# emilk/field_interpolation

Measured on AMD Instinct MI355X. Metric: solved lattice points/sec (assembly+CG to field within 1e-5 of the CPU reference by the solver's estimate: ended at rel. residual 1.1e-08), higher is better.
Workload: dtype f64

## Files before the change

field_interpolation_amd/_capi.py:

```python
import ctypes as C
import os

HERE = os.path.dirname(os.path.abspath(__file__))
LIB_PATH = os.environ.get("FI_HIP_LIB", os.path.join(HERE, "libfi_hip.so"))

FI_OK = 0
FI_HOST, FI_DEVICE = 0, 1
FI_F32, FI_F64 = 0, 1
ERR_NAMES = {1: "FI_ERR_INVALID", 2: "FI_ERR_HIP", 3: "FI_ERR_STATE", 4: "FI_ERR_COMM",
             5: "FI_ERR_UNSUPPORTED", 6: "FI_ERR_BREAKDOWN", 7: "FI_ERR_TIMEOUT"}

SYMBOLS = [
    "fi_last_error", "fi_device_count", "fi_ctx_create", "fi_ctx_create_slab", "fi_ctx_destroy",
    "fi_slab_range", "fi_slab_point_range", "fi_slab_partition", "fi_halo_width", "fi_comm_unique_id", "fi_comm_init", "fi_comm_init_host", "fi_comm_info", "fi_comm_self_test", "fi_set_model", "fi_add_points", "fi_add_border_prior",
    "fi_add_rows_coo", "fi_assemble", "fi_clear_points", "fi_set_option", "fi_solve_cg", "fi_jacobi", "fi_tile_pass", "fi_error_map",
    "fi_get_solution_f64", "fi_true_residual", "fi_apply_AtA_f64", "fi_get_Atb_f64", "fi_get_diag_f64",
    "fi_get_stats", "fi_memory_pool", "fi_time_apply", "fi_upscale_field",
    "fi_group_create", "fi_group_destroy", "fi_group_size", "fi_group_rank", "fi_group_assemble",
    "fi_group_solve_cg", "fi_group_apply_AtA_f64", "fi_group_true_residual", "fi_group_get_solution_f64", "fi_group_tile_pass", "fi_group_error_map",
    "fi_group_iso_extract", "fi_iso_extract", "fi_iso_extract_field", "fi_mesh_info", "fi_mesh_copy", "fi_mesh_destroy",
    "fi_dual_contour", "fi_dual_contour_field",
    "fi_mesh_create", "fi_mesh_parts", "fi_mesh_measure", "fi_mesh_select", "fi_mesh_simplify",
    "fi_mesh_smooth", "fi_mesh_normals", "fi_mesh_sample", "fi_mesh_deviation", "fi_mesh_register", "fi_points_register",
    "fi_group_sample", "fi_sample", "fi_sample_field",
    "fi_nearest", "fi_distance_field", "fi_points_create", "fi_points_nearest", "fi_points_distance_field", "fi_points_destroy",
    "fi_knn", "fi_points_knn", "fi_estimate_normals", "fi_points_estimate_normals",
    "fi_orient_normals", "fi_points_orient_normals",
    "fi_radius_count", "fi_points_radius_count", "fi_neighbour_distances", "fi_points_neighbour_distances",
    "fi_outliers_statistical", "fi_points_outliers_statistical", "fi_outliers_radius", "fi_points_outliers_radius", "fi_cloud_thin",
    "fi_cluster", "fi_points_cluster", "fi_cluster_measure", "fi_plane_fit", "fi_planes_segment",
    "fi_points_describe", "fi_feature_match", "fi_align_correspondences",
    "fi_surface_create", "fi_surface_from_mesh", "fi_surface_distance", "fi_surface_distance_field", "fi_surface_destroy",
    "fi_surface_raycast", "fi_surface_count_hits", "fi_surface_contains", "fi_surface_signed_distance",
    "fi_surface_signed_distance_field",
    "fi_redistance", "fi_redistance_field",
    "fi_point_count", "fi_point_residuals", "fi_robust_reweight", "fi_reset_point_weights", "fi_solve_robust",
]
FI_LOSS = {"huber": 0, "cauchy": 1, "tukey": 2}
FI_LOSS_NONE = -1
FI_REGISTER = {"plane": 0, "point": 1}
FI_THIN = {"mean": 0, "first": 1}


class FiWeights(C.Structure):
    _fields_ = [("data_pos", C.c_float), ("data_gradient", C.c_float),
                ("model_0", C.c_float), ("model_1", C.c_float), ("model_2", C.c_float),
                ("model_3", C.c_float), ("model_4", C.c_float), ("gradient_smoothness", C.c_float),
                ("value_kernel", C.c_int), ("gradient_kernel", C.c_int)]


class FiSolveOptions(C.Structure):
    _fields_ = [("tile", C.c_int), ("tile_size", C.c_int), ("cg", C.c_int),
                ("max_iterations", C.c_int), ("error_tolerance", C.c_float)]


class FiTriplet(C.Structure):
    _fields_ = [("row", C.c_int), ("col", C.c_int), ("value", C.c_float)]


class FiStats(C.Structure):
    _fields_ = [("num_unknowns", C.c_long), ("num_data_rows", C.c_long), ("num_cells", C.c_long),
                ("num_generic_rows", C.c_long), ("iterations", C.c_int), ("converged", C.c_int),
                ("rel_residual", C.c_double), ("assemble_ms", C.c_double), ("solve_ms", C.c_double),
                ("spmv_ms_avg", C.c_double), ("spmv_samples", C.c_int), ("spmv_bytes", C.c_double),
                ("restarts", C.c_int), ("verified_residual", C.c_double),
                ("num_levels", C.c_int), ("coarse_iterations", C.c_int),
                ("prec_ms_avg", C.c_double), ("prec_samples", C.c_int), ("prec_bytes", C.c_double),
                ("operator_applies", C.c_int), ("halo_exchanges", C.c_int), ("reductions", C.c_int),
                ("coarse_unconverged", C.c_int), ("field_estimate", C.c_double), ("field_per_residual", C.c_double),
                ("stop_residual", C.c_double), ("field_rounds", C.c_int)]


class FiRobustOptions(C.Structure):
    _fields_ = [("loss", C.c_int), ("tuning", C.c_float), ("scale", C.c_float), ("rounds", C.c_int),
                ("weight_tolerance", C.c_float)]


class FiRobustStats(C.Structure):
    _fields_ = [("rounds", C.c_int), ("iterations", C.c_int), ("scale", C.c_float), ("max_weight_change", C.c_float),
                ("points_used", C.c_long), ("points_zeroed", C.c_long), ("reweight_ms", C.c_double)]


class FiMeshPart(C.Structure):
    _fields_ = [("vertices", C.c_longlong), ("primitives", C.c_longlong), ("edges", C.c_longlong),
                ("boundary", C.c_longlong), ("irregular", C.c_longlong), ("size", C.c_double), ("enclosed", C.c_double),
                ("lo", C.c_float * 3), ("hi", C.c_float * 3)]


class FiSmoothOptions(C.Structure):
    _fields_ = [("iterations", C.c_int), ("lam", C.c_float), ("mu", C.c_float), ("boundary", C.c_int),
                ("max_move", C.c_float), ("normals", C.c_int)]


class FiDeviation(C.Structure):
    _fields_ = [("queries", C.c_longlong), ("counted", C.c_longlong), ("beyond", C.c_longlong), ("invalid", C.c_longlong),
                ("at", C.c_longlong), ("max", C.c_double), ("mean", C.c_double), ("rms", C.c_double), ("where", C.c_float * 3)]


class FiRegisterOptions(C.Structure):
    _fields_ = [("mode", C.c_int), ("max_iterations", C.c_int), ("max_distance", C.c_float), ("rotation_tolerance", C.c_double),
# ... 8 lines not shown


class FiOutlierStats(C.Structure):
    _fields_ = [("counted", C.c_long), ("kept", C.c_long), ("mean", C.c_double), ("stddev", C.c_double), ("threshold", C.c_double)]


class FiClusterStats(C.Structure):
    _fields_ = [("clusters", C.c_long), ("core", C.c_long), ("border", C.c_long), ("noise", C.c_long), ("non_finite", C.c_long)]


class FiClusterRow(C.Structure):
    _fields_ = [("count", C.c_long), ("core", C.c_long), ("lo", C.c_float * 3), ("hi", C.c_float * 3), ("centroid", C.c_double * 3)]


class FiPlaneOptions(C.Structure):
    _fields_ = [("threshold", C.c_float), ("max_trials", C.c_long), ("confidence", C.c_double), ("refine", C.c_int),
                ("seed", C.c_ulonglong), ("axis", C.c_float * 3), ("min_cos", C.c_float)]


class FiPlaneModel(C.Structure):
    _fields_ = [("found", C.c_int), ("refits", C.c_int), ("inliers", C.c_long), ("candidates", C.c_long), ("trials", C.c_long),
                ("normal", C.c_double * 3), ("offset", C.c_double), ("rms", C.c_double)]


class FiAlignOptions(C.Structure):
    _fields_ = [("threshold", C.c_float), ("similarity", C.c_float), ("max_trials", C.c_long), ("confidence", C.c_double),
                ("seed", C.c_ulonglong)]


class FiAlignment(C.Structure):
    _fields_ = [("found", C.c_int), ("pairs", C.c_long), ("live", C.c_long), ("trials", C.c_long), ("valid", C.c_long),
                ("inliers", C.c_long), ("transform", C.c_double * 16), ("rms", C.c_double)]


class FiError(RuntimeError):
    def __init__(self, code, msg):
        super().__init__("%s: %s" % (ERR_NAMES.get(code, "error %d" % code), msg))
        self.code = code


_LIB = None


def lib():
    global _LIB
    if _LIB is not None:
        return _LIB
    if not os.path.exists(LIB_PATH):
        raise ImportError("field_interpolation_amd: %s is missing -- run `python -m field_interpolation_amd.build` "
                          "(hipcc, gfx950).  There is no CPU fallback." % LIB_PATH)
    L = C.CDLL(LIB_PATH)
    vp, ip, fp, dp = C.c_void_p, C.POINTER(C.c_int), C.c_void_p, C.POINTER(C.c_double)
    L.fi_last_error.restype = C.c_char_p
    L.fi_device_count.argtypes = [ip]
    L.fi_ctx_create.argtypes = [C.POINTER(vp), C.c_int, ip, C.c_int]
    L.fi_ctx_create_slab.argtypes = [C.POINTER(vp), C.c_int, ip, C.c_int, C.c_int, C.c_int]
    L.fi_ctx_destroy.argtypes = [vp]
    L.fi_slab_range.argtypes = [vp, ip, ip]
    L.fi_slab_point_range.argtypes = [vp, C.POINTER(C.c_float), C.POINTER(C.c_float)]
    L.fi_slab_partition.argtypes = [C.c_int, C.c_int, C.c_int, ip, ip]
    L.fi_halo_width.argtypes = [C.POINTER(FiWeights), ip]
    L.fi_comm_unique_id.argtypes = [vp]
    L.fi_comm_init.argtypes = [vp, vp]
    L.fi_comm_info.argtypes = [vp, C.POINTER(C.c_long)]
    L.fi_comm_init_host.argtypes = [vp, C.c_char_p, C.c_int]
    L.fi_set_model.argtypes = [vp, C.POINTER(FiWeights)]
    L.fi_add_points.argtypes = [vp, C.c_long, fp, fp, fp, fp, C.c_float, C.c_int, C.c_float, C.c_int, C.c_int]
    L.fi_add_border_prior.argtypes = [vp, C.c_float]
    L.fi_add_rows_coo.argtypes = [vp, C.c_long, C.c_long, vp, fp, C.c_int]
    L.fi_assemble.argtypes = [vp]
    L.fi_clear_points.argtypes = [vp]
    L.fi_solve_cg.argtypes = [vp, fp, C.c_int, C.c_float, fp, ip, C.POINTER(C.c_float), C.c_int]
    L.fi_set_option.argtypes = [vp, C.c_int, C.c_double]
    L.fi_jacobi.argtypes = [vp, fp, C.c_int, C.c_float, fp, C.c_int]
    L.fi_tile_pass.argtypes = [vp, fp, C.c_int, fp, C.c_int]
    L.fi_comm_self_test.argtypes = [C.c_int, C.c_long]
    L.fi_error_map.argtypes = [vp, fp, fp, C.c_int]
    L.fi_get_solution_f64.argtypes = [vp, dp]
    L.fi_true_residual.argtypes = [vp, dp]
    L.fi_apply_AtA_f64.argtypes = [vp, dp, dp]
    L.fi_get_Atb_f64.argtypes = [vp, dp]
    L.fi_get_diag_f64.argtypes = [vp, dp]
    L.fi_get_stats.argtypes = [vp, C.POINTER(FiStats)]
    L.fi_time_apply.argtypes = [vp, C.c_int, dp]
    L.fi_memory_pool.argtypes = [C.c_longlong, C.POINTER(C.c_longlong)]
    L.fi_upscale_field.argtypes = [fp, C.c_int, ip, ip, fp, C.c_int]
    L.fi_group_create.argtypes = [C.POINTER(vp), C.c_int, ip, C.c_int, C.c_int]
    L.fi_group_destroy.argtypes = [vp]
    L.fi_group_size.argtypes = [vp]
    L.fi_group_rank.restype = vp
    L.fi_group_rank.argtypes = [vp, C.c_int]
    L.fi_group_assemble.argtypes = [vp]
    L.fi_group_solve_cg.argtypes = [vp, fp, C.c_int, C.c_float, fp, ip, C.POINTER(C.c_float)]
    L.fi_group_apply_AtA_f64.argtypes = [vp, dp, dp]
    L.fi_group_true_residual.argtypes = [vp, dp]
    L.fi_group_get_solution_f64.argtypes = [vp, dp]
    L.fi_group_tile_pass.argtypes = [vp, fp, C.c_int, fp]
    L.fi_group_error_map.argtypes = [vp, fp, fp]
    L.fi_group_iso_extract.argtypes = [vp, fp, C.c_float, C.POINTER(vp)]
    L.fi_iso_extract.argtypes = [vp, fp, C.c_float, C.c_int, C.POINTER(vp)]
    L.fi_iso_extract_field.argtypes = [fp, C.c_int, ip, C.c_float, C.c_int, C.POINTER(vp)]
    L.fi_dual_contour.argtypes = [vp, fp, fp, C.c_float, C.c_int, C.POINTER(vp)]
    L.fi_dual_contour_field.argtypes = [fp, fp, C.c_int, ip, C.c_float, C.c_int, C.POINTER(vp)]
    L.fi_mesh_info.argtypes = [vp, C.POINTER(C.c_long), C.POINTER(C.c_long), ip]
    L.fi_mesh_copy.argtypes = [vp, fp, fp, vp, vp, C.c_int]
    L.fi_mesh_destroy.argtypes = [vp]
    L.fi_mesh_create.argtypes = [C.POINTER(vp), C.c_int, C.c_long, fp, fp, vp, C.c_long, vp, C.c_int]
    L.fi_mesh_parts.argtypes = [vp, C.POINTER(C.c_long), vp, vp, C.c_int]
    L.fi_mesh_measure.argtypes = [vp, C.c_long, vp, C.POINTER(C.c_long)]
    L.fi_mesh_select.argtypes = [vp, C.c_long, vp, C.POINTER(vp)]
    L.fi_mesh_simplify.argtypes = [vp, C.c_float, vp, C.c_int, vp, C.c_int, C.POINTER(vp)]
    L.fi_mesh_smooth.argtypes = [vp, C.POINTER(FiSmoothOptions), C.POINTER(vp)]
    L.fi_mesh_normals.argtypes = [vp, C.POINTER(vp)]
    L.fi_mesh_sample.argtypes = [vp, C.c_long, C.c_ulonglong, C.c_int, fp, fp, vp, C.c_int]
    L.fi_mesh_deviation.argtypes = [vp, vp, C.c_long, C.c_ulonglong, C.c_float, C.POINTER(FiDeviation), C.POINTER(FiDeviation), fp,
                                    C.c_int]
    L.fi_mesh_register.argtypes = [vp, vp, C.c_long, fp, C.POINTER(FiRegisterOptions), dp, C.POINTER(FiRegistration), fp, fp, C.c_int]
    L.fi_points_register.argtypes = [vp, fp, C.c_long, fp, C.POINTER(FiRegisterOptions), dp, C.POINTER(FiRegistration), fp, fp,
                                     C.c_int]
    L.fi_group_sample.argtypes = [vp, fp, C.c_long, fp, C.c_int, C.c_float, fp, fp]
    L.fi_sample.argtypes = [vp, fp, C.c_long, fp, C.c_int, C.c_float, fp, fp, C.c_int]
    L.fi_sample_field.argtypes = [fp, C.c_int, ip, C.c_long, fp, C.c_int, C.c_float, fp, fp, C.c_int]
    L.fi_nearest.argtypes = [vp, C.c_long, fp, C.c_float, fp, vp, C.c_int]
    L.fi_distance_field.argtypes = [vp, C.c_float, fp, vp, C.c_int]
    L.fi_points_create.argtypes = [C.POINTER(vp), C.c_int, C.c_long, fp, C.c_int]
    L.fi_points_nearest.argtypes = [vp, C.c_long, fp, C.c_float, fp, vp, C.c_int]
    L.fi_points_distance_field.argtypes = [vp, ip, C.c_float, fp, vp, C.c_int]
    L.fi_points_destroy.argtypes = [vp]
    L.fi_knn.argtypes = [vp, C.c_long, fp, C.c_int, C.c_float, fp, vp, C.c_int]
    L.fi_points_knn.argtypes = [vp, C.c_long, fp, C.c_int, C.c_float, fp, vp, C.c_int]
    L.fi_estimate_normals.argtypes = [vp, C.c_int, C.c_float, C.c_int, fp, C.c_long, fp, fp, C.c_int]
    L.fi_points_estimate_normals.argtypes = [vp, C.c_int, C.c_float, C.c_int, fp, C.c_long, fp, fp, C.c_int]
    L.fi_orient_normals.argtypes = [vp, C.c_int, C.c_float, C.c_int, fp, C.c_long, fp, vp, C.c_int]
    L.fi_points_orient_normals.argtypes = [vp, C.c_int, C.c_float, C.c_int, fp, C.c_long, fp, vp, C.c_int]
    L.fi_radius_count.argtypes = [vp, C.c_long, fp, C.c_float, C.c_int, vp, C.c_int]
    L.fi_points_radius_count.argtypes = [vp, C.c_long, fp, C.c_float, C.c_int, vp, C.c_int]
    L.fi_neighbour_distances.argtypes = [vp, C.c_int, C.c_float, fp, fp, vp, C.c_int]
    L.fi_points_neighbour_distances.argtypes = [vp, C.c_int, C.c_float, fp, fp, vp, C.c_int]
    L.fi_outliers_statistical.argtypes = [vp, C.c_int, C.c_float, C.c_float, vp, C.POINTER(FiOutlierStats), C.c_int]
    L.fi_points_outliers_statistical.argtypes = [vp, C.c_int, C.c_float, C.c_float, vp, C.POINTER(FiOutlierStats), C.c_int]
    L.fi_outliers_radius.argtypes = [vp, C.c_float, C.c_int, vp, C.POINTER(C.c_long), C.c_int]
    L.fi_points_outliers_radius.argtypes = [vp, C.c_float, C.c_int, vp, C.POINTER(C.c_long), C.c_int]
    L.fi_cloud_thin.argtypes = [C.c_int, C.c_long, fp, fp, fp, C.c_float, C.POINTER(C.c_float), C.c_int, fp, fp, fp, vp, vp, vp,
                                C.POINTER(C.c_long), C.c_int]
    L.fi_cluster.argtypes = [vp, C.c_float, C.c_int, vp, vp, C.POINTER(FiClusterStats), C.c_int]
    L.fi_points_cluster.argtypes = [vp, C.c_float, C.c_int, vp, vp, C.POINTER(FiClusterStats), C.c_int]
    L.fi_cluster_measure.argtypes = [C.c_int, C.c_long, fp, vp, vp, C.c_long, C.POINTER(FiClusterRow), C.c_int]
    L.fi_plane_fit.argtypes = [C.c_int, C.c_long, fp, vp, C.POINTER(FiPlaneOptions), C.POINTER(FiPlaneModel), vp, C.c_int]
    L.fi_planes_segment.argtypes = [C.c_int, C.c_long, fp, vp, C.POINTER(FiPlaneOptions), C.c_int, C.c_long, vp,
                                    C.POINTER(FiPlaneModel), ip, C.c_int]
    L.fi_points_describe.argtypes = [vp, fp, C.c_int, C.c_float, fp, vp, C.c_int]
    L.fi_feature_match.argtypes = [C.c_int, C.c_long, fp, vp, C.c_long, fp, vp, vp, fp, C.c_int]
    L.fi_align_correspondences.argtypes = [C.c_long, fp, C.c_long, fp, C.c_long, vp, vp, C.POINTER(FiAlignOptions),
                                           C.POINTER(FiAlignment), vp, C.c_int]
    L.fi_surface_create.argtypes = [C.POINTER(vp), C.c_int, C.c_long, fp, C.c_long, vp, C.c_int]
    L.fi_surface_from_mesh.argtypes = [C.POINTER(vp), vp]
    L.fi_surface_distance.argtypes = [vp, C.c_long, fp, C.c_float, fp, vp, fp, C.c_int]
    L.fi_surface_distance_field.argtypes = [vp, ip, C.c_float, fp, vp, C.c_int]
    L.fi_surface_destroy.argtypes = [vp]
    L.fi_surface_raycast.argtypes = [vp, C.c_long, fp, fp, C.c_float, C.c_float, fp, vp, fp, C.c_int]
    L.fi_surface_count_hits.argtypes = [vp, C.c_long, fp, fp, C.c_float, C.c_float, C.c_int, vp, C.c_int]
    L.fi_surface_contains.argtypes = [vp, C.c_long, fp, C.POINTER(C.c_float), vp, C.c_int]
    L.fi_surface_signed_distance.argtypes = [vp, C.c_long, fp, C.c_float, fp, vp, fp, C.c_int]
    L.fi_surface_signed_distance_field.argtypes = [vp, ip, C.c_float, fp, vp, C.c_int]
    L.fi_redistance.argtypes = [vp, fp, C.c_float, C.c_int, C.c_float, fp, vp, C.POINTER(vp), C.c_int]
    L.fi_redistance_field.argtypes = [fp, C.c_int, ip, C.c_float, C.c_int, C.c_float, fp, vp, C.POINTER(vp), C.c_int]
# ... 27 lines not shown
```

field_interpolation_amd/api.py:

```python
import collections
import ctypes as C
import enum
import math

import numpy as np

from . import _capi
from ._capi import FI_DEVICE, FI_F32, FI_F64, FI_HOST, FiError, FiStats, FiWeights, check

MAX_DIM = 3


class ValueKernel(enum.IntEnum):
    kNearestNeighbor = 0
    kLinearInterpolation = 1


class GradientKernel(enum.IntEnum):
    kNearestNeighbor = 0
    kCellEdges = 1
    kLinearInterpolation = 2


class Weights:
# ... 1654 lines not shown
    def set_cheb_smoother(self, degree=0, ratio=0.0):
        check(_capi.lib().fi_set_option(self._h, 14, float(degree)))
        check(_capi.lib().fi_set_option(self._h, 15, float(ratio)))
        self._dirty = True

    def set_kcycle(self, levels):
        check(_capi.lib().fi_set_option(self._h, 13, float(levels)))
        self._dirty = True

    def set_polynomial(self, terms, ratio=None):
        check(_capi.lib().fi_set_option(self._h, 6, float(terms)))
        if ratio is not None:
            check(_capi.lib().fi_set_option(self._h, 7, float(ratio)))

    def set_mg_smoother(self, polynomial=True, safe_factor=None, terms=None, ratio=None):
        check(_capi.lib().fi_set_option(self._h, 8, 1.0 if polynomial else 0.0))
        if safe_factor is not None:
            check(_capi.lib().fi_set_option(self._h, 9, float(safe_factor)))
        if terms is not None:
            check(_capi.lib().fi_set_option(self._h, 10, float(terms)))
        if ratio is not None:
            check(_capi.lib().fi_set_option(self._h, 11, float(ratio)))
        self._dirty = True

    def jacobi(self, guess, num_iterations, weight):
        self._ready()
        g, kg, _kg = _buf(guess)
        out = self._out(guess)
        o, ko, _ko = _buf(out)
        check(_capi.lib().fi_jacobi(self._h, g, int(num_iterations), float(weight), o, _same_memory(kg, ko)))
        return out

    def error_map(self, solution):
        self._ready()
        g, kg, _kg = _buf(solution)
        out = self._out(solution)
        o, ko, _ko = _buf(out)
        check(_capi.lib().fi_error_map(self._h, g, o, _same_memory(kg, ko)))
        return out

    def tile_pass(self, guess, tile_size=16):
        self._ready()
        g, kg, _kg = _buf(guess)
        out = self._out(guess)
        o, ko, _ko = _buf(out)
        check(_capi.lib().fi_tile_pass(self._h, g, int(tile_size), o, _same_memory(kg, ko)))
        return out

    def solution_f64(self):
        out = np.empty(self.num_owned, np.float64)
        check(_capi.lib().fi_get_solution_f64(self._h, out.ctypes.data_as(C.POINTER(C.c_double))))
        return out

    def true_residual(self):
        r = C.c_double(0)
        check(_capi.lib().fi_true_residual(self._h, C.byref(r)))
        return r.value

    def apply_AtA(self, x):
        self._ready()
        xx = np.ascontiguousarray(x, np.float64)
        y = np.empty(self.num_owned, np.float64)
        dp = C.POINTER(C.c_double)
        check(_capi.lib().fi_apply_AtA_f64(self._h, xx.ctypes.data_as(dp), y.ctypes.data_as(dp)))
        return y

    def Atb(self):
        self._ready()
        out = np.empty(self.num_owned, np.float64)
        check(_capi.lib().fi_get_Atb_f64(self._h, out.ctypes.data_as(C.POINTER(C.c_double))))
        return out

    def diag(self):
        self._ready()
        out = np.empty(self.num_owned, np.float64)
        check(_capi.lib().fi_get_diag_f64(self._h, out.ctypes.data_as(C.POINTER(C.c_double))))
        return out

    def stats(self):
        s = FiStats()
        check(_capi.lib().fi_get_stats(self._h, C.byref(s)))
        return {name: getattr(s, name) for name, _ in FiStats._fields_}

    def time_apply(self, reps=20):
        self._ready()
        ms = C.c_double(0)
        check(_capi.lib().fi_time_apply(self._h, reps, C.byref(ms)))
        return ms.value


class LatticeGroup:

    def __init__(self, sizes, nranks, dtype="f32"):
        self.sizes = [int(s) for s in sizes]
        self.dtype = dtype
        self._g = C.c_void_p()
        sz = (C.c_int * len(self.sizes))(*self.sizes)
        check(_capi.lib().fi_group_create(C.byref(self._g), len(self.sizes), sz, {"f32": FI_F32, "f64": FI_F64}[dtype],
                                          nranks))
        self.members = [LatticeField(self.sizes, dtype=dtype, rank=r, nranks=nranks,
                                     _borrowed=_capi.lib().fi_group_rank(self._g, r)) for r in range(nranks)]

    def __del__(self):
        g = getattr(self, "_g", None)
        if g and _capi._LIB is not None:
            for m in getattr(self, "members", []):
                m._h = None
            _capi._LIB.fi_group_destroy(g)
            self._g = None

    @property
    def num_unknowns(self):
        return int(np.prod(self.sizes))

    def add_field_constraints(self, weights):
        for m in self.members:
            m.add_field_constraints(weights)

    def add_points(self, *a, **kw):
        for m in self.members:
            m.add_points(*a, **kw)

    def set_levels(self, levels, coarse_tolerance=None):
        for m in self.members:
            m.set_levels(levels, coarse_tolerance)

    def set_multigrid(self, on=True):
        for m in self.members:
            m.set_multigrid(on)

    def set_mixed_precision(self, on=True):
        for m in self.members:
            m.set_mixed_precision(on)

    def set_field_tolerance(self, tol):
        for m in self.members:
            m.set_field_tolerance(tol)

    def set_polynomial(self, terms, ratio=None):
        for m in self.members:
            m.set_polynomial(terms, ratio)

    def set_mg_smoother(self, polynomial=True, safe_factor=None, terms=None, ratio=None):
        for m in self.members:
            m.set_mg_smoother(polynomial, safe_factor, terms, ratio)

    def set_cheb_smoother(self, degree=0, ratio=0.0):
        for m in self.members:
            m.set_cheb_smoother(degree, ratio)

    def set_kcycle(self, levels):
        for m in self.members:
            m.set_kcycle(levels)

    def assemble(self):
        check(_capi.lib().fi_group_assemble(self._g))
        for m in self.members:
            m._dirty = False

    def apply_AtA(self, x):
        xx = np.ascontiguousarray(x, np.float64)
        y = np.empty(self.num_unknowns, np.float64)
        dp = C.POINTER(C.c_double)
        check(_capi.lib().fi_group_apply_AtA_f64(self._g, xx.ctypes.data_as(dp), y.ctypes.data_as(dp)))
        return y

# ... 184 lines not shown
```

field_interpolation_amd/csrc/fi_capi.hip:

```cpp
#include "fi_solver_internal.h"
#include "fi_stage.h"
#include "fi_workers.h"
#include "fi_iso.h"
#include "fi_dual.h"
#include "fi_sample.h"
#include "fi_nearest.h"
#include "fi_knn.h"
#include "fi_orient.h"
#include "fi_surface.h"
#include "fi_ray.h"
#include "fi_robust.h"
#include "fi_parts.h"
#include "fi_simplify.h"
#include "fi_smooth.h"
#include "fi_meshpts.h"
#include "fi_register.h"
#include "fi_cloud.h"
#include "fi_cluster.h"
#include "fi_plane.h"
#include "fi_align.h"
#include "fi_feature.h"

#include <memory>

// ... 4 lines not shown
void set_error(const char* fmt, ...)
{
	char    buf[1024];
	va_list ap;
	va_start(ap, fmt);
	vsnprintf(buf, sizeof(buf), fmt, ap);
	va_end(ap);
	g_error = buf;
}


namespace {
struct UpscaleArgs {
	int ndim;
	int ssz[3], lsz[3];
};
__global__ __launch_bounds__(kThreads) void k_upscale(UpscaleArgs a, int64_t nlarge, const float* __restrict__ small,
                                                       float* __restrict__ out)
{
	const int64_t li = static_cast<int64_t>(blockIdx.x) * kThreads + threadIdx.x;
	if (li >= nlarge) { return; }
	int     base[3];
	float   t[3];
	int64_t rest = li;
	for (int d = 0; d < a.ndim; ++d) {
		const int c = static_cast<int>(rest % a.lsz[d]);
		rest /= a.lsz[d];
		const float sp = static_cast<float>(c) * (static_cast<float>(a.ssz[d]) - 1.0f) /
		                 (static_cast<float>(a.lsz[d]) - 1.0f);
		const bool  ok = sp == sp;
		const float fl = floorf(sp);
		base[d] = ok ? static_cast<int>(fl) : -4;
		t[d]    = ok ? sp - static_cast<float>(base[d]) : 0.0f;
	}
	float wsum = 0.0f, fsum = 0.0f;
	for (int q = 0; q < (1 << a.ndim); ++q) {
		int64_t idx = 0, stride = 1;
		float   w  = 1.0f;
		bool    in = true;
		for (int d = 0; d < a.ndim; ++d) {
			const int up = (q >> d) & 1;
			const int cc = base[d] + up;
			idx += stride * cc;
			stride *= a.ssz[d];
			w *= up ? t[d] : 1.0f - t[d];
			in = in && (0 <= cc) && (cc < a.ssz[d]);
		}
		if (in) {
			wsum += w;
			fsum += w * small[idx];
		}
	}
	out[li] = (wsum == 0.0f) ? 0.0f : fsum / wsum;
}

int64_t lattice_points(int ndim, const int* sizes)
{
	int64_t n = 1;
	for (int d = 0; d < ndim; ++d) {
		FI_REQUIRE(sizes[d] >= 1, FI_ERR_INVALID, "sizes[%d] = %d", d, sizes[d]);
		n *= sizes[d];
	}
	return n;
}

template <typename Handle>
int destroy_handle(Handle* h)
{
	if (!h) { return FI_OK; }
	int dev = 0;
	const bool switched = hipGetDevice(&dev) == hipSuccess && dev != h->device && hipSetDevice(h->device) == hipSuccess;
	delete h;
	if (switched) { (void)hipSetDevice(dev); }
	return FI_OK;
}

}

void check_ctx(const fi_ctx* c) { FI_REQUIRE(c != nullptr, FI_ERR_INVALID, "null context"); }

void check_assembled(const fi_ctx* c)
{
	check_ctx(c);
	FI_REQUIRE(c->assembled, FI_ERR_STATE, "fi_assemble has not been called");
}

void bind_device(const fi_ctx* c) { FI_HIP_TRY(hipSetDevice(c->device)); }

fi_ctx* create_ctx(int ndim, const int* sizes, int dtype, int rank, int nranks)
{
	FI_REQUIRE(1 <= ndim && ndim <= FI_MAX_DIM, FI_ERR_INVALID, "ndim must be 1..%d (got %d)", FI_MAX_DIM, ndim);
	FI_REQUIRE(sizes != nullptr, FI_ERR_INVALID, "sizes is null");
	FI_REQUIRE(dtype == FI_F32 || dtype == FI_F64, FI_ERR_INVALID, "unknown dtype %d", dtype);
	FI_REQUIRE(nranks >= 1 && 0 <= rank && rank < nranks, FI_ERR_INVALID, "bad rank %d of %d", rank, nranks);
	int64_t n = 1;
	for (int d = 0; d < ndim; ++d) {
		FI_REQUIRE(sizes[d] >= 1, FI_ERR_INVALID, "sizes[%d] = %d", d, sizes[d]);
		n *= sizes[d];
		FI_REQUIRE(static_cast<int64_t>(sizes[d]) + 1 < (1 << 20), FI_ERR_INVALID, "sizes[%d] too large", d);
	}
	FI_REQUIRE(n < (1LL << 31), FI_ERR_UNSUPPORTED, "lattice has %lld unknowns; the reference indexes with int",
	           static_cast<long long>(n));
	FI_REQUIRE(nranks == 1 || sizes[ndim - 1] >= nranks, FI_ERR_INVALID, "fewer planes (%d) than ranks (%d)",
	           sizes[ndim - 1], nranks);
	auto* c = new fi_ctx();
	try {
		c->dtype  = dtype;
		c->rank   = rank;
		c->nranks = nranks;
		FI_HIP_TRY(hipGetDevice(&c->device));
		c->stream = stream_take();
		c->halo = 1;
		c->stats.field_estimate = -1.0;
		compute_geom(c, ndim, sizes);
		c->scal.alloc(3 * sizeof(CgScalars));
		FI_HIP_TRY(hipMemset(c->scal.p, 0, 2 * sizeof(CgScalars)));
		c->scal_host = static_cast<CgScalars*>(pinned_take(sizeof(CgScalars), &c->scal_host_cap));
		c->w = fi_weights{1.0f, 1.0f, 0.0f, 0.0f, 0.5f, 0.0f, 0.0f, 0.0f, FI_VALUE_LINEAR_INTERPOLATION,
		                  FI_GRADIENT_CELL_EDGES};
	} catch (...) {
		fi_ctx_destroy(c);
		throw;
	}
	return c;
}


}


extern "C" {

const char* fi_last_error(void) { return fi::g_error.c_str(); }

int fi_device_count(int* count)
{
	FI_API_BEGIN
	FI_REQUIRE(count != nullptr, FI_ERR_INVALID, "count is null");
	int n = 0;
	const hipError_t e = hipGetDeviceCount(&n);
	*count = (e == hipSuccess) ? n : 0;
	FI_API_END
}

int fi_ctx_create(fi_ctx** out, int ndim, const int* sizes, int dtype)
{
	FI_API_BEGIN
	FI_REQUIRE(out != nullptr, FI_ERR_INVALID, "out is null");
	*out = fi::create_ctx(ndim, sizes, dtype, 0, 1);
	FI_API_END
}

int fi_ctx_create_slab(fi_ctx** out, int ndim, const int* sizes, int dtype, int rank, int nranks)
{
	FI_API_BEGIN
	FI_REQUIRE(out != nullptr, FI_ERR_INVALID, "out is null");
	*out = fi::create_ctx(ndim, sizes, dtype, rank, nranks);
	FI_API_END
}

int fi_ctx_destroy(fi_ctx* c)
{
	if (!c) { return FI_OK; }
	(void)hipSetDevice(c->device);
	bool drained = true;
	for (hipStream_t st : {c->stream, c->level_stream, c->level_stream2, c->build_stream, c->comm_stream}) {
		if (st && hipStreamSynchronize(st) != hipSuccess) { drained = false; }
	}
	struct Quiescent {
		bool was;
		explicit Quiescent(bool ok) : was(fi::pool_quiescent) { fi::pool_quiescent = ok; }
		~Quiescent() { fi::pool_quiescent = was; }
	} quiescent(drained);
	for (auto* pb : c->pending) { delete pb; }
	for (auto* pb : c->pending_pool) { delete pb; }
	for (auto* b : c->batches) { delete b; }
	for (auto* b : c->batches_pool) { delete b; }
	if (c->coarse) { fi_ctx_destroy(c->coarse); }
	if (c->twin) { fi_ctx_destroy(c->twin); }
	c->pending.clear();
	c->pending_pool.clear();
	for (auto e : c->ev) { (void)hipEventDestroy(e); }
	for (auto e : c->ev_prec) { (void)hipEventDestroy(e); }
	fi::stream_give(c->level_stream, drained);
	if (c->ev_level) { (void)hipEventDestroy(c->ev_level); }
	fi::stream_give(c->level_stream2, drained);
	if (c->build_stream) {
		fi::stream_give(c->build_stream, drained);
		(void)hipEventDestroy(c->ev_build);
	}
	if (c->ev_level2) { (void)hipEventDestroy(c->ev_level2); }
	if (c->comm_stream) {
		fi::stream_give(c->comm_stream, drained);
		(void)hipEventDestroy(c->ev_ready);
		(void)hipEventDestroy(c->ev_halo);
	}
	if (c->comm && c->owns_comm) { fi::comm_destroy(c->comm); }
	if (c->scal_host) {
		if (drained) { fi::pinned_give(c->scal_host, c->scal_host_cap); } else { (void)hipHostFree(c->scal_host); }
	}
	for (int s = 0; s < 3; ++s) {
		if (!c->pin[s]) { continue; }
		if (drained) { fi::pinned_give(c->pin[s], c->pin_bytes[s]); } else { (void)hipHostFree(c->pin[s]); }
	}
	if (c->ev_unwatched) { (void)hipEventDestroy(c->ev_unwatched); }
	if (c->ev_asm0) {
		(void)hipEventDestroy(c->ev_asm0);
		(void)hipEventDestroy(c->ev_asm1);
	}
	if (c->stream && c->owns_stream) { fi::stream_give(c->stream, drained); }
	fi::nearest_release(c);
	delete c;
	return FI_OK;
}

int fi_memory_pool(long long keep_bytes, long long* cached_bytes)
{
	FI_API_BEGIN
	const size_t keep = keep_bytes < 0 ? ~size_t(0) : static_cast<size_t>(keep_bytes);
	const size_t left = fi::pool_trim(keep);
	if (keep == 0) {
		fi::forget_iterations();
		fi::forget_lambdas();
	}
	if (cached_bytes) { *cached_bytes = static_cast<long long>(left); }
	FI_API_END
}

int fi_slab_partition(int planes, int rank, int nranks, int* lo, int* hi)
{
	FI_API_BEGIN
	FI_REQUIRE(nranks >= 1 && 0 <= rank && rank < nranks && planes >= 0, FI_ERR_INVALID, "bad slab request");
	if (lo) { *lo = static_cast<int>(static_cast<int64_t>(rank) * planes / nranks); }
	if (hi) { *hi = static_cast<int>(static_cast<int64_t>(rank + 1) * planes / nranks); }
	FI_API_END
}

int fi_halo_width(const fi_weights* w, int* width)
{
	FI_API_BEGIN
	FI_REQUIRE(w && width, FI_ERR_INVALID, "null argument");
	const int reach = fi::model_reach(*w);
	*width = reach > 1 ? reach : 1;
	FI_API_END
}

int fi_slab_range(const fi_ctx* c, int* lo, int* hi)
{
	FI_API_BEGIN
	fi::check_ctx(c);
	if (lo) { *lo = c->slab_lo; }
	if (hi) { *hi = c->slab_hi; }
	FI_API_END
}

int fi_slab_point_range(const fi_ctx* c, float* lo, float* hi)
{
	FI_API_BEGIN
	fi::check_ctx(c);
	const int L = c->levels_wanted > 0 ? c->levels_wanted : 0;
	int first_tail = 0;
	const int nlevels = fi::plan_levels(c, &first_tail);
	if (c->nranks > 1 && first_tail <= nlevels) {
		if (lo) { *lo = -std::numeric_limits<float>::max(); }
		if (hi) { *hi = std::numeric_limits<float>::max(); }
		return FI_OK;
	}
	const float cell = static_cast<float>(1 << (L < 20 ? L : 20));
	if (lo) { *lo = static_cast<float>(c->slab_lo) - 2.0f * cell; }
	if (hi) { *hi = static_cast<float>(c->slab_hi) + (L > 0 ? 2.0f : 1.0f) * cell; }
	FI_API_END
}

int fi_set_model(fi_ctx* c, const fi_weights* w)
{
	FI_API_BEGIN
	fi::check_ctx(c);
	FI_REQUIRE(w != nullptr, FI_ERR_INVALID, "weights is null");
	c->w         = *w;
	c->model_set = true;
	c->assembled = false;
	for (fi_ctx* l = c; l; l = l->coarse) { l->poly_lambda = 0; }
	if (c->twin) {
		for (fi_ctx* l = c->twin; l; l = l->coarse) { l->poly_lambda = 0; }
	}
	FI_API_END
}

int fi_add_points(fi_ctx* c, long n, const float* positions, const float* normals, const float* point_weights,
                  const float* values, float value_weight, int value_kernel, float gradient_weight, int gradient_kernel,
                  int memory)
{
	FI_API_BEGIN
	fi::check_ctx(c);
	fi::bind_device(c);
	FI_REQUIRE(n >= 0, FI_ERR_INVALID, "negative point count");
	if (n == 0) { return FI_OK; }
	FI_REQUIRE(positions != nullptr, FI_ERR_INVALID, "positions is null");
	FI_REQUIRE(value_kernel == FI_VALUE_NEAREST_NEIGHBOR || value_kernel == FI_VALUE_LINEAR_INTERPOLATION,
	           FI_ERR_INVALID, "Unknown value kernel: %d", value_kernel);
	FI_REQUIRE(!(value_kernel == FI_VALUE_NEAREST_NEIGHBOR && normals == nullptr), FI_ERR_INVALID,
	           "nearest-neighbour value kernel needs normals (field_interpolation.cpp:361)");
	if (normals) {
		FI_REQUIRE(gradient_kernel >= 0 && gradient_kernel <= 2, FI_ERR_INVALID, "Unknown gradient kernel: %d",
		           gradient_kernel);
	}
	fi::check_memory(memory);
	const int D = c->g.ndim;
	fi::DevBuf dpos, dnrm, dpw, dval;
	const float *p = positions, *g = normals, *w = point_weights, *v = values;
	if (memory == FI_HOST) {
		auto up = [&](fi::DevBuf& b, const float* src, size_t count) -> const float* {
			if (!src) { return nullptr; }
			b.alloc(sizeof(float) * count);
			FI_HIP_TRY(hipMemcpyAsync(b.p, src, sizeof(float) * count, hipMemcpyHostToDevice, c->stream));
			return b.as<float>();
		};
		p = up(dpos, positions, static_cast<size_t>(n) * D);
		g = up(dnrm, normals, static_cast<size_t>(n) * D);
		w = up(dpw, point_weights, static_cast<size_t>(n));
		v = up(dval, values, static_cast<size_t>(n));
	}
	fi::nearest_release(c);
	fi::add_points_device(c, n, p, g, w, v, value_weight, value_kernel, gradient_weight, gradient_kernel);
	c->assembled = false;
	FI_API_END
}

}

namespace fi {
void add_points_device(fi_ctx* c, long n, const float* p, const float* g, const float* w, const float* v, float value_weight,
                       int value_kernel, float gradient_weight, int gradient_kernel)
{
	const int D = c->g.ndim;
	{
		fi::PointBatch* b = nullptr;
		if (!c->batches_pool.empty()) {
			b = c->batches_pool.back();
			c->batches_pool.pop_back();
		} else {
			b = new fi::PointBatch();
		}
		c->batches.push_back(b);
		auto keep = [&](fi::DevBuf& dst, const float* src, size_t count) {
			if (!src) { return false; }
			dst.alloc(sizeof(float) * count);
			FI_HIP_TRY(hipMemcpyAsync(dst.p, src, sizeof(float) * count, hipMemcpyDeviceToDevice, c->stream));
			return true;
		};
		b->n = n;
		b->prior = false;
		b->reweighted = false;
		b->had_pw     = false;
		c->robust.n   = 0;
		keep(b->pos, p, static_cast<size_t>(n) * D);
		b->has_nrm = keep(b->nrm, g, static_cast<size_t>(n) * D);
		b->has_pw  = keep(b->pw, w, static_cast<size_t>(n));
		b->has_val = keep(b->val, v, static_cast<size_t>(n));
		b->vw = value_weight;
		b->gw = gradient_weight;
		b->vk = value_kernel;
		b->gk = gradient_kernel;
	}
	const bool lin = g && gradient_kernel == FI_GRADIENT_LINEAR_INTERPOLATION;
	fi::emit_point_rows(c, n, p, g, w, v, value_weight, value_kernel, lin ? 0.0f : gradient_weight,
	                    lin ? FI_GRADIENT_CELL_EDGES : gradient_kernel);
	if (lin && gradient_weight != 0.0f) { fi::generic_add_gradient_linear(c, n, p, g, w, gradient_weight); }
	FI_HIP_TRY(hipStreamSynchronize(c->stream));
}
}

extern "C" {

int fi_add_border_prior(fi_ctx* c, float weight)
{
	FI_API_BEGIN
	fi::check_ctx(c);
	fi::bind_device(c);
	if (weight == 0.0f) { return FI_OK; }
	FI_REQUIRE(c->nranks == 1, FI_ERR_UNSUPPORTED, "fi_add_border_prior on a slab context: a rank sees only its own points");
	bool any = false;
	for (const fi::PointBatch* b : c->batches) { any = any || (b->n > 0 && !b->prior); }
	FI_REQUIRE(any, FI_ERR_STATE, "fi_add_border_prior needs the data points: call it after fi_add_points");
	fi::DevBuf pos, val, zero;
	const int64_t nb = fi::border_prior_points(c, pos, val);
	if (nb > 0) {
		zero.alloc(sizeof(float) * nb * c->g.ndim);
		FI_HIP_TRY(hipMemsetAsync(zero.p, 0, sizeof(float) * nb * c->g.ndim, c->stream));
		fi::add_points_device(c, static_cast<long>(nb), pos.as<float>(), zero.as<float>(), nullptr, val.as<float>(), weight,
		                      FI_VALUE_NEAREST_NEIGHBOR, 0.0f, FI_GRADIENT_NEAREST_NEIGHBOR);
		c->batches.back()->prior = true;
	}
	c->assembled = false;
	FI_API_END
}

int fi_add_rows_coo(fi_ctx* c, long nrows, long ntriplets, const fi_triplet* triplets, const float* rhs, int memory)
{
	FI_API_BEGIN
	fi::check_ctx(c);
	fi::bind_device(c);
	FI_REQUIRE(nrows >= 0 && ntriplets >= 0, FI_ERR_INVALID, "negative count");
	fi::check_memory(memory);
	FI_REQUIRE(c->nranks == 1, FI_ERR_UNSUPPORTED, "generic rows need an undivided lattice");
	FI_REQUIRE((ntriplets == 0 || triplets) && (nrows == 0 || rhs), FI_ERR_INVALID, "null buffer");
	fi::generic_add_coo(c, nrows, ntriplets, triplets, rhs, memory);
	c->assembled = false;
	FI_API_END
}

int fi_clear_points(fi_ctx* c)
{
	FI_API_BEGIN
	fi::check_ctx(c);
	for (auto* pb : c->pending) { c->pending_pool.push_back(pb); }
	c->pending.clear();
	for (auto* b : c->batches) { c->batches_pool.push_back(b); }
	c->batches.clear();
	c->robust.n = 0;
	fi::nearest_release(c);
	fi::generic_clear(c);
	c->assembled = false;
	FI_API_END
}

namespace fi {
void finish_assemble_timing(fi_ctx* c)
{
	if (!c->asm_time_pending) { return; }
	c->asm_time_pending = false;
	if (hipEventSynchronize(c->ev_asm1) != hipSuccess) { return; }
	float ms = 0;
	if (hipEventElapsedTime(&ms, c->ev_asm0, c->ev_asm1) == hipSuccess) { c->stats.assemble_ms = ms; }
}
}

int fi_assemble(fi_ctx* c)
{
	FI_API_BEGIN
	fi::check_ctx(c);
	fi::bind_device(c);
	fi::finish_assemble_timing(c);
	if (!c->ev_asm0) {
		FI_HIP_TRY(hipEventCreate(&c->ev_asm0));
		FI_HIP_TRY(hipEventCreate(&c->ev_asm1));
	}
	const hipEvent_t e0 = c->ev_asm0, e1 = c->ev_asm1;
	fi::chain_mark(nullptr);
	FI_HIP_TRY(hipEventRecord(e0, c->stream));
	{
		bool trip = c->generic.ntrip != 0, grad = !fi::holds_value_rows_only(c);
		if (c->facts_forced) {
			trip = c->forced_trip;
			grad = c->forced_grad;
		} else if (c->nranks > 1 && fi::comm_ready(c)) {
			double* slot = (c->scal.as<fi::CgScalars>() + 2)->sums;
			double  v[2] = {trip ? 1.0 : 0.0, grad ? 1.0 : 0.0};
			FI_HIP_TRY(hipMemcpyAsync(slot, v, sizeof(v), hipMemcpyHostToDevice, c->stream));
			fi::allreduce_sum(c, slot, 2);
			FI_HIP_TRY(hipMemcpyAsync(v, slot, sizeof(v), hipMemcpyDeviceToHost, c->stream));
			FI_HIP_TRY(hipStreamSynchronize(c->stream));
			trip = v[0] > 0.0;
			grad = v[1] > 0.0;
		}
		c->any_trip        = trip;
		c->value_rows_only = !grad && !trip;
		c->facts_forced    = false;
	}
	const int reach = fi::model_reach(c->w);
	const int want_reach = reach > 1 ? reach : 1;
	int want_halo = want_reach;
	if (c->nranks > 1 && c->g.ndim == 3 && c->poly_terms >= 3 && c->poly_terms <= 5 && !c->any_trip &&
	    !fi::test_switch("FI_NO_DEEP_HALO")) {
		const int deep = 2 * (c->poly_terms - 1);
		const int thinnest = c->g.gn[2] / c->nranks;
		if (deep > want_halo && thinnest >= deep) { want_halo = deep; }
	}
	if (c->nranks > 1 && c->g.ndim == 3 && c->mg_mode == 1 && c->mg_smoother == 1 && c->levels_wanted > 0 && c->value_rows_only &&
	    !c->any_trip && (c->dtype == FI_F32 || c->mixed) && c->mg_terms >= 3 && c->mg_terms <= 5 &&
	    !(c->w.model_3 > 0 || c->w.model_4 > 0 || c->w.gradient_smoothness > 0) && !fi::test_switch("FI_NO_DEEP_HALO") &&
	    !fi::test_switch("FI_MG_FULL_SMOOTHER")) {
		const int deep = 2 * (c->mg_terms - 1);
		const int thinnest = c->g.gn[2] / c->nranks;
		if (deep > want_halo && thinnest >= deep) { want_halo = deep; }
	}
	c->min_slab = c->nranks > 1 ? c->g.gn[c->g.ndim - 1] / c->nranks : c->g.gn[c->g.ndim - 1];
	if (c->nranks > 1 && (want_halo != c->halo || want_reach != c->reach)) {
		c->halo  = want_halo;
		c->reach = want_reach;
		int sizes[3] = {c->g.gn[0], c->g.gn[1], c->g.gn[2]};
		fi::compute_geom(c, c->g.ndim, sizes);
		c->vectors_ready = false;
		c->vectors_stale = true;
	}
	if (c->nranks > 1) {
		FI_REQUIRE(c->slab_hi - c->slab_lo >= c->reach, FI_ERR_UNSUPPORTED,
		           "slab of %d planes is thinner than the stencil reach %d", c->slab_hi - c->slab_lo, c->reach);
	}
	const bool mixed64 = c->mixed && c->dtype == FI_F64;
	c->want_lump = mixed64 && fi::lumped_twin_wanted(c);
	const bool beside = (c->levels_wanted > 0 || mixed64) && !c->any_trip && !fi::test_switch("FI_SERIAL_LEVELS");
	if (beside && mixed64) {
		const int keep = c->levels_wanted;
		c->levels_wanted = 0;
		fi::build_levels(c);
		c->levels_wanted = keep;
	}
	if (beside) {
		if (!c->level_stream) {
			c->level_stream = fi::stream_take();
			FI_HIP_TRY(hipEventCreateWithFlags(&c->ev_level, hipEventDisableTiming));
		}
		FI_HIP_TRY(hipEventRecord(c->ev_level, c->stream));
		FI_HIP_TRY(hipStreamWaitEvent(c->level_stream, c->ev_level, 0));
		int         helper_code = FI_OK;
		std::string helper_msg;
		if (mixed64) {
			fi::twin_prepare(c);
			if (!c->level_stream2) {
				c->level_stream2 = fi::stream_take();
				FI_HIP_TRY(hipEventCreateWithFlags(&c->ev_level2, hipEventDisableTiming));
			}
			FI_HIP_TRY(hipStreamWaitEvent(c->level_stream2, c->ev_level, 0));
		}
		auto guarded = [&](auto&& work, int* code, std::string* msg) {
			try {
				FI_HIP_TRY(hipSetDevice(c->device));
				fi::AllocStream none(nullptr);
				work();
			} catch (const fi::Fail& f) {
				*code = f.code;
				*msg  = fi_last_error();
			} catch (...) {
				*code = FI_ERR_HIP;
				*msg  = "unexpected exception while building the coarser levels";
			}
		};
		const bool lumped = mixed64 && c->twin && c->twin->lumped;
		auto build = [&]() {
			guarded([&]() {
				if (lumped) {
				} else if (mixed64) {
					fi::twin_assemble(c, c->level_stream);
				} else {
					fi::build_levels(c, nullptr, c->level_stream);
				}
			}, &helper_code, &helper_msg);
		};
		int         helper2_code = FI_OK;
		std::string helper2_msg;
		auto build2 = [&]() {
			guarded([&]() { fi::build_levels(c->twin, c, c->level_stream2); }, &helper2_code, &helper2_msg);
		};
		fi::Worker *helper = nullptr, *helper2 = nullptr;
		try {
			if (!lumped) {
				helper = fi::worker_pool().acquire();
				helper->run(build);
			}
			if (mixed64) {
				helper2 = fi::worker_pool().acquire();
				helper2->run(build2);
			}
		} catch (...) {
		}
		int main_code = FI_OK;
		c->defer_scaling_exchange = true;
		try {
			fi::AllocStream alloc_on(c->stream);
			fi::chain_mark("threads started");
			fi::assemble(c);
			fi::chain_mark("finest: rows assembled");
			fi::generic_assemble(c);
			fi::stencil_prepare(c);
			fi::chain_mark("finest: stencil prepared");
			fi::operator_prepare(c);
			fi::chain_mark("finest: operator prepared");
		} catch (const fi::Fail& f) {
			main_code = f.code;
		} catch (...) {
			main_code = FI_ERR_HIP;
			fi::set_error("unexpected exception while assembling the finest level");
		}
		if (lumped && main_code == FI_OK) {
			try {
				fi::AllocStream alloc_on(c->stream);
				c->twin->defer_scaling_exchange = true;
				fi::twin_assemble_lumped(c);
				fi::chain_mark("finest: lumped replica");
			} catch (const fi::Fail& f) {
				main_code = f.code;
			} catch (...) {
				main_code = FI_ERR_HIP;
				fi::set_error("unexpected exception while building the lumped replica");
			}
		}
		if (helper) {
			helper->wait();
			fi::worker_pool().release(helper);
		} else if (main_code == FI_OK && !lumped) {
			build();
		}
		if (mixed64) {
			if (helper2) {
				helper2->wait();
				fi::worker_pool().release(helper2);
			} else if (main_code == FI_OK) {
				build2();
			}
			if (helper_code == FI_OK && helper2_code != FI_OK) {
				helper_code = helper2_code;
				helper_msg  = helper2_msg;
			}
		}
		fi::chain_mark("helpers joined");
		fi_ctx* const first_built = mixed64 ? c->twin : c->coarse;
		for (fi_ctx* l = first_built; l; l = l->coarse) { l->stream = c->stream; }
		const bool mine_ok = main_code == FI_OK && helper_code == FI_OK;
		bool peers_ok = true;
		try {
			peers_ok = fi::all_ranks_ok(c, mine_ok);
		} catch (const fi::Fail&) {
			peers_ok = false;
		}
		if (!mine_ok || !peers_ok) {
			(void)hipStreamSynchronize(c->level_stream);
			if (c->level_stream2) { (void)hipStreamSynchronize(c->level_stream2); }
			c->defer_scaling_exchange = false;
			if (main_code != FI_OK) { throw fi::Fail{main_code}; }
			if (helper_code != FI_OK) {
				fi::set_error("%s", helper_msg.c_str());
				throw fi::Fail{helper_code};
			}
			fi::set_error("fi_assemble: another rank failed while assembling its slab");
			throw fi::Fail{FI_ERR_COMM};
		}
		if (fi::tuning_switch("FI_ASM_CHAIN_TIMES")) {
			hipEvent_t a = nullptr, b = nullptr, d = nullptr;
			FI_HIP_TRY(hipEventCreate(&a));
			FI_HIP_TRY(hipEventCreate(&b));
			FI_HIP_TRY(hipEventCreate(&d));
			FI_HIP_TRY(hipEventRecord(a, c->stream));
			FI_HIP_TRY(hipEventRecord(b, c->level_stream));
			if (mixed64) { FI_HIP_TRY(hipEventRecord(d, c->level_stream2)); }
			FI_HIP_TRY(hipEventSynchronize(a));
			FI_HIP_TRY(hipEventSynchronize(b));
			if (mixed64) { FI_HIP_TRY(hipEventSynchronize(d)); }
			float ta = 0, tb = 0, td = 0;
			(void)hipEventElapsedTime(&ta, e0, a);
			(void)hipEventElapsedTime(&tb, e0, b);
			if (mixed64) { (void)hipEventElapsedTime(&td, e0, d); }
			std::fprintf(stderr, "fi_assemble chains: solver stream %.3f ms, level stream %.3f ms, second level stream %.3f ms\n", ta, tb, td);
			(void)hipEventDestroy(a);
			(void)hipEventDestroy(b);
			(void)hipEventDestroy(d);
		}
		FI_HIP_TRY(hipEventRecord(c->ev_level, c->level_stream));
		FI_HIP_TRY(hipStreamWaitEvent(c->stream, c->ev_level, 0));
		if (mixed64) {
			FI_HIP_TRY(hipEventRecord(c->ev_level2, c->level_stream2));
			FI_HIP_TRY(hipStreamWaitEvent(c->stream, c->ev_level2, 0));
			fi::twin_finish(c);
		}
		fi::operator_finish_ghosts(c);
		for (fi_ctx* l = first_built; l; l = l->coarse) { fi::operator_finish_ghosts(l); }
	} else {
	fi::AllocStream alloc_on(c->stream);
	fi::assemble(c);
	fi::generic_assemble(c);
	fi::stencil_prepare(c);
	fi::operator_prepare(c);
	}
	if (beside) {
		if (!mixed64) { fi::build_twin(c); }
	} else if (mixed64) {
		const int keep = c->levels_wanted;
		c->levels_wanted = 0;
		fi::build_levels(c);
		c->levels_wanted = keep;
		fi::build_twin(c);
	} else {
		fi::build_levels(c);
		fi::build_twin(c);
	}
	FI_HIP_TRY(hipEventRecord(e1, c->stream));
	fi::chain_mark("fi_assemble returns");
	c->asm_time_pending   = true;
	c->stats.assemble_ms  = 0.0;
	c->stats.num_levels   = 1;
	for (fi_ctx* l = c->coarse; l; l = l->coarse) { c->stats.num_levels += 1; }
	if (c->twin) { c->stats.num_levels = c->twin->stats.num_levels; }
	c->stats.num_unknowns = c->g.nown;
	c->stats.spmv_bytes   = fi::apply_algorithmic_bytes(c);
	c->assembled          = true;
	c->vectors_ready      = false;
	FI_API_END
}

int fi_solve_cg(fi_ctx* c, const float* guess, int max_iterations, float tol, float* out, int* iterations,
                float* rel_residual, int memory)
{
	FI_API_BEGIN
	fi::check_assembled(c);
	fi::bind_device(c);
	fi::check_memory(memory);
	fi::AllocStream alloc_on(c->stream);
	if (c->dtype == FI_F64) {
		fi::solve_cg_t<double>(c, guess, max_iterations, tol, out, iterations, rel_residual, memory);
	} else {
		fi::solve_cg_t<float>(c, guess, max_iterations, tol, out, iterations, rel_residual, memory);
	}
	FI_API_END
}

int fi_set_option(fi_ctx* c, int option, double value)
{
	FI_API_BEGIN
	fi::check_ctx(c);
	switch (option) {
	case FI_OPT_VERIFY_RESIDUAL: c->verify_residual = value != 0.0; break;
	case FI_OPT_LEVELS:
		c->levels_wanted = value > 0 ? static_cast<int>(value) : 0;
		c->assembled = false;
		break;
	case FI_OPT_COARSE_TOLERANCE: c->coarse_tol = value > 0 ? value : 1e-3; break;
	case FI_OPT_MULTIGRID: c->mg_mode = value != 0.0 ? 1 : 0; break;
	case FI_OPT_MIXED_PRECISION:
		FI_REQUIRE(value == 0.0 || c->dtype == FI_F64, FI_ERR_INVALID, "FI_OPT_MIXED_PRECISION needs an FI_F64 context");
		c->mixed = value != 0.0 ? 1 : 0;
		c->assembled = false;
		break;
	case FI_OPT_POLY_TERMS:
		FI_REQUIRE(value >= 0 && value <= 32, FI_ERR_INVALID, "FI_OPT_POLY_TERMS must be 0..32");
		c->poly_terms = static_cast<int>(value);
		break;
	case FI_OPT_POLY_RATIO:
		FI_REQUIRE(value > 1.0 && value <= 1000.0, FI_ERR_INVALID, "FI_OPT_POLY_RATIO must be in (1, 1000]");
		c->poly_ratio = value;
		break;
	case FI_OPT_MG_SMOOTHER:
		c->mg_smoother = value != 0.0 ? 1 : 0;
		c->assembled = false;
		break;
	case FI_OPT_MG_SAFE_FACTOR:
		FI_REQUIRE(value >= 1.0 && value <= 64.0, FI_ERR_INVALID, "FI_OPT_MG_SAFE_FACTOR must be 1..64");
		c->mg_safe = value;
		c->assembled = false;
		break;
	case FI_OPT_MG_TERMS:
		FI_REQUIRE(value >= 2 && value <= 16, FI_ERR_INVALID, "FI_OPT_MG_TERMS must be 2..16");
		c->mg_terms = static_cast<int>(value);
		c->assembled = false;
		break;
	case FI_OPT_MG_RATIO:
		FI_REQUIRE(value > 1.0 && value <= 1000.0, FI_ERR_INVALID, "FI_OPT_MG_RATIO must be in (1, 1000]");
		c->mg_pratio = value;
		c->assembled = false;
		break;
	case FI_OPT_MG_CHEB_DEGREE:
		FI_REQUIRE(value == 0 || (value >= 2 && value <= 16), FI_ERR_INVALID, "FI_OPT_MG_CHEB_DEGREE must be 0 or 2..16");
		c->mg_cheb_degree = static_cast<int>(value);
		c->assembled = false;
		break;
	case FI_OPT_MG_CHEB_RATIO:
		FI_REQUIRE(value == 0 || (value > 1.0 && value <= 1000.0), FI_ERR_INVALID, "FI_OPT_MG_CHEB_RATIO must be 0 or in (1, 1000]");
		c->mg_cheb_ratio = value;
		c->assembled = false;
		break;
	case FI_OPT_MG_KCYCLE:
		FI_REQUIRE(value >= 0 && value <= 16, FI_ERR_INVALID, "FI_OPT_MG_KCYCLE must be 0..16");
		c->mg_kcycle = static_cast<int>(value);
		c->assembled = false;
		break;
	case FI_OPT_FIELD_TOLERANCE:
		FI_REQUIRE(value >= 0.0 && value < 1.0, FI_ERR_INVALID, "FI_OPT_FIELD_TOLERANCE must be in [0, 1)");
		c->field_tol = value;
		break;
	default: FI_REQUIRE(false, FI_ERR_INVALID, "unknown option %d", option);
	}
	FI_API_END
}

int fi_jacobi(fi_ctx* c, const float* guess, int num_iterations, float weight, float* out, int memory)
{
	FI_API_BEGIN
	fi::check_assembled(c);
	fi::bind_device(c);
	fi::check_memory(memory);
	if (num_iterations < 0) { num_iterations = 0; }
	if (c->dtype == FI_F64) {
		fi::jacobi_t<double>(c, guess, num_iterations, weight, out, memory);
	} else {
		fi::jacobi_t<float>(c, guess, num_iterations, weight, out, memory);
	}
	FI_API_END
}

int fi_error_map(fi_ctx* c, const float* solution, float* out, int memory)
{
	FI_API_BEGIN
	fi::check_assembled(c);
	fi::bind_device(c);
	fi::check_memory(memory);
	FI_REQUIRE(solution && out, FI_ERR_INVALID, "fi_error_map needs a solution and an output buffer");
	fi::ensure_vectors(c);
	fi::RankSet R{c};
	if (c->dtype == FI_F64) {
		fi::load_owned<double>(c, c->x, solution, memory);
		fi::halo_exchange(R, &fi_ctx::x);
		fi::error_map(c, c->x.p, c->q.p);
		fi::store_owned<double>(c, c->q, out, memory);
	} else {
		fi::load_owned<float>(c, c->x, solution, memory);
		fi::halo_exchange(R, &fi_ctx::x);
		fi::error_map(c, c->x.p, c->q.p);
		fi::store_owned<float>(c, c->q, out, memory);
	}
	FI_API_END
}

int fi_point_count(const fi_ctx* c, long* n)
{
	FI_API_BEGIN
	fi::check_ctx(c);
	FI_REQUIRE(n != nullptr, FI_ERR_INVALID, "null output");
	*n = fi::robust_point_count(c);
	FI_API_END
}

int fi_point_residuals(fi_ctx* c, const float* field, float* residuals, int memory)
{
	FI_API_BEGIN
	fi::check_ctx(c);
	fi::bind_device(c);
	fi::check_memory(memory);
	fi::robust_residuals(c, field, residuals, memory);
	FI_API_END
}

int fi_robust_reweight(fi_ctx* c, const float* field, const fi_robust_options* options, float* omega, float* scale, int memory)
{
	FI_API_BEGIN
	fi::check_ctx(c);
	fi::bind_device(c);
	FI_REQUIRE(options != nullptr, FI_ERR_INVALID, "options is null");
	fi::check_memory(memory);
	const fi::RobustStep step = fi::robust_reweight(c, field, options->loss, options->tuning, options->scale, omega, memory);
	if (scale) { *scale = step.scale; }
	FI_API_END
}

int fi_reset_point_weights(fi_ctx* c)
{
	FI_API_BEGIN
	fi::check_ctx(c);
	fi::bind_device(c);
	fi::robust_reset(c);
	FI_API_END
}

int fi_solve_robust(fi_ctx* c, const float* guess, const fi_robust_options* options, int max_iterations, float tol, float* out,
                    float* omega, fi_robust_stats* stats, int memory)
{
	FI_API_BEGIN
	fi::check_ctx(c);
	fi::bind_device(c);
	FI_REQUIRE(options != nullptr, FI_ERR_INVALID, "options is null");
	fi::check_memory(memory);
	FI_REQUIRE(options->rounds >= 0, FI_ERR_INVALID, "rounds = %d", options->rounds);
	FI_REQUIRE(options->weight_tolerance >= 0.0f, FI_ERR_INVALID, "weight_tolerance must be >= 0");
	const long n = fi::robust_check(c);
	fi_robust_stats rs{};
	if (stats) { *stats = rs; }
	auto ok = [](int code) {
		if (code != FI_OK) { throw fi::Fail{code}; }
	};
	if (!c->assembled) { ok(fi_assemble(c)); }
	int it = 0;
	ok(fi_solve_cg(c, guess, max_iterations, tol, out, &it, nullptr, memory));
	rs.iterations = it;
	struct Start {
		fi_ctx* c;
		~Start() { c->guess_native = nullptr; }
	} start{c};
	const size_t es = fi::elem_size(c);
	bool weighted = false;
	for (int round = 0; round < options->rounds; ++round) {
		const auto t0 = std::chrono::steady_clock::now();
		c->robust.xkeep.alloc(es * c->g.nown);
		FI_HIP_TRY(hipMemcpyAsync(c->robust.xkeep.p, static_cast<const char*>(c->x.p) + es * c->g.own_first, es * c->g.nown,
		                          hipMemcpyDeviceToDevice, c->stream));
		const fi::RobustStep step = fi::robust_reweight(c, nullptr, options->loss, options->tuning, options->scale, nullptr, memory);
		rs.reweight_ms += std::chrono::duration<double, std::milli>(std::chrono::steady_clock::now() - t0).count();
		rs.scale             = step.scale;
		rs.max_weight_change = step.max_weight_change;
		rs.points_used       = step.points_used;
		rs.points_zeroed     = step.points_zeroed;
		if (step.scale == 0.0f) { break; }
		weighted = true;
		ok(fi_assemble(c));
		c->guess_native = c->robust.xkeep.p;
		const int code = fi_solve_cg(c, nullptr, max_iterations, tol, out, &it, nullptr, memory);
		c->guess_native = nullptr;
		ok(code);
		rs.iterations += it;
		rs.rounds = round + 1;
		if (options->weight_tolerance > 0.0f && step.max_weight_change < options->weight_tolerance) { break; }
	}
	if (omega) {
		if (weighted || c->robust.n == n) {
			FI_HIP_TRY(hipMemcpy(omega, c->robust.omega.p, sizeof(float) * n, memory == FI_HOST ? hipMemcpyDeviceToHost : hipMemcpyDeviceToDevice));
		} else {
			std::vector<float> ones(static_cast<size_t>(n), 1.0f);
			FI_HIP_TRY(hipMemcpy(omega, ones.data(), sizeof(float) * n, memory == FI_HOST ? hipMemcpyHostToHost : hipMemcpyHostToDevice));
		}
	}
	if (stats) { *stats = rs; }
	FI_API_END
}

int fi_tile_pass(fi_ctx* c, const float* guess, int tile_size, float* out, int memory)
{
	FI_API_BEGIN
	fi::check_assembled(c);
	fi::bind_device(c);
	fi::check_memory(memory);
	FI_REQUIRE(tile_size >= 2, FI_ERR_INVALID, "tile_size %d < 2 (sparse_linear.cpp:254)", tile_size);
	FI_REQUIRE(guess && out, FI_ERR_INVALID, "fi_tile_pass needs a guess and an output buffer");
	FI_REQUIRE(c->nranks == 1 || c->generic.ntrip == 0, FI_ERR_UNSUPPORTED, "the tile pre-solver over triplet rows needs an undivided lattice");
	if (c->dtype == FI_F64) {
		fi::tile_pass_t<double>(c, guess, tile_size, out, memory);
	} else {
		fi::tile_pass_t<float>(c, guess, tile_size, out, memory);
	}
	FI_API_END
}

int fi_get_solution_f64(fi_ctx* c, double* out)
{
	FI_API_BEGIN
	fi::check_assembled(c);
	fi::bind_device(c);
	FI_REQUIRE(c->vectors_ready && out, FI_ERR_STATE, "no solution yet");
	c->dtype == FI_F64 ? fi::get_vec_f64_t<double>(c, c->x, out) : fi::get_vec_f64_t<float>(c, c->x, out);
	FI_API_END
}

int fi_true_residual(fi_ctx* c, double* rel)
{
	FI_API_BEGIN
	fi::check_assembled(c);
	fi::bind_device(c);
	FI_REQUIRE(rel != nullptr, FI_ERR_INVALID, "null output");
	*rel = c->dtype == FI_F64 ? fi::true_residual_t<double>(c) : fi::true_residual_t<float>(c);
	FI_API_END
}

int fi_apply_AtA_f64(fi_ctx* c, const double* x, double* y)
{
	FI_API_BEGIN
	fi::check_assembled(c);
	fi::bind_device(c);
	FI_REQUIRE(x && y, FI_ERR_INVALID, "null vector");
	c->dtype == FI_F64 ? fi::apply_f64_t<double>(c, x, y) : fi::apply_f64_t<float>(c, x, y);
	FI_API_END
}

int fi_get_Atb_f64(fi_ctx* c, double* out)
{
	FI_API_BEGIN
	fi::check_assembled(c);
	fi::bind_device(c);
	c->dtype == FI_F64 ? fi::get_vec_f64_t<double>(c, c->atb, out) : fi::get_vec_f64_t<float>(c, c->atb, out);
	FI_API_END
}

int fi_get_diag_f64(fi_ctx* c, double* out)
{
	FI_API_BEGIN
	fi::check_assembled(c);
	fi::bind_device(c);
	c->dtype == FI_F64 ? fi::get_vec_f64_t<double>(c, c->diag, out) : fi::get_vec_f64_t<float>(c, c->diag, out);
	FI_API_END
}

int fi_get_stats(const fi_ctx* c, fi_stats* out)
{
	FI_API_BEGIN
	fi::check_ctx(c);
	FI_REQUIRE(out != nullptr, FI_ERR_INVALID, "null output");
	fi::finish_assemble_timing(const_cast<fi_ctx*>(c));
	*out = c->stats;
	out->coarse_unconverged = 0;
	const fi_ctx* top = c->twin && c->twin->coarse ? c->twin : c;
	for (const fi_ctx* l = top->coarse; l; l = l->coarse) {
		if (!l->unwatched_pending || !l->ev_unwatched || !l->pin[2]) { continue; }
		if (hipEventSynchronize(l->ev_unwatched) != hipSuccess) { continue; }
		const fi::CgScalars* was = static_cast<const fi::CgScalars*>(l->pin[2]);
		const bool met = was->done == 1 || was->done == 5 || was->done == 4;
		if (!met) { out->coarse_unconverged += 1; }
		out->coarse_iterations += (met ? was->iter : l->unwatched_expected) - l->unwatched_expected;
	}
	FI_API_END
}

int fi_time_apply(fi_ctx* c, int reps, double* ms_per_launch)
{
	FI_API_BEGIN
	fi::check_assembled(c);
	fi::bind_device(c);
	FI_REQUIRE(reps > 0 && ms_per_launch, FI_ERR_INVALID, "bad arguments");
	fi::ensure_vectors(c);
	fi::CgScalars init{};
	FI_HIP_TRY(hipMemcpyAsync(c->scal.p, &init, sizeof(init), hipMemcpyHostToDevice, c->stream));
	fi::EventPair timer;
	const hipEvent_t e0 = timer.e0, e1 = timer.e1;
	const char* which = fi::tuning_switch("FI_TIME_STEP");
	const int   step = which ? atoi(which) : 0;
	auto launch = [&]() {
		if (step >= 1 && fi::stencil_cheb_available(c)) {
			c->dtype == FI_F64 ? fi::ensure_poly_vectors<double>(c) : fi::ensure_poly_vectors<float>(c);
			if (step == 1) {
				fi::stencil_cheb_step(c, c->r.p, nullptr, c->r.p, c->mg_d.p, 0.3, 0.2, c->partial.as<double>(), 0, 0.0, 0.5);
			} else if (step == 2) {
				fi::stencil_cheb_step(c, c->mg_d.p, c->mg_x.p, c->r.p, c->mg_x.p, 0.3, 0.2, c->partial.as<double>(), 0, 0.5);
			} else {
				fi::stencil_cheb_step(c, c->mg_x.p, c->mg_d.p, c->r.p, c->mg_d.p, 0.3, 0.2, c->partial.as<double>());
			}
		} else {
			fi::apply_AtA(c, c->p.p, c->q.p, c->partial.as<double>());
		}
	};
	launch();
	FI_HIP_TRY(hipEventRecord(e0, c->stream));
	for (int k = 0; k < reps; ++k) { launch(); }
	FI_HIP_TRY(hipEventRecord(e1, c->stream));
	FI_HIP_TRY(hipEventSynchronize(e1));
	float ms = 0;
	FI_HIP_TRY(hipEventElapsedTime(&ms, e0, e1));
	*ms_per_launch = ms / reps;
	FI_API_END
}

int fi_upscale_field(const float* small_field, int ndim, const int* small_sizes, const int* large_sizes, float* out,
                     int memory)
{
	FI_API_BEGIN
	FI_REQUIRE(small_field && small_sizes && large_sizes && out, FI_ERR_INVALID, "null argument");
	FI_REQUIRE(1 <= ndim && ndim <= FI_MAX_DIM, FI_ERR_INVALID, "ndim must be 1..3");
	fi::check_memory(memory);
	fi::UpscaleArgs a{};
	a.ndim = ndim;
	int64_t ns = 1, nl = 1;
	for (int d = 0; d < ndim; ++d) {
		FI_REQUIRE(small_sizes[d] >= 1 && large_sizes[d] >= 1, FI_ERR_INVALID, "bad size");
		a.ssz[d] = small_sizes[d];
		a.lsz[d] = large_sizes[d];
		ns *= small_sizes[d];
		nl *= large_sizes[d];
	}
	fi::stage::In<float>  s(small_field, ns, memory, nullptr);
	fi::stage::Out<float> o(out, nl, memory);
	hipLaunchKernelGGL(fi::k_upscale, dim3(fi::blocks_for(nl)), dim3(fi::kThreads), 0, nullptr, a, nl, s.dev, o.dev);
	FI_HIP_TRY(hipGetLastError());
	o.back(nullptr);
	FI_HIP_TRY(hipDeviceSynchronize());
	FI_API_END
}


int fi_iso_extract(fi_ctx* c, const float* field, float iso, int memory, fi_mesh** out)
{
	FI_API_BEGIN
	fi::check_ctx(c);
	FI_REQUIRE(out != nullptr, FI_ERR_INVALID, "out is null");
	*out = nullptr;
	fi::bind_device(c);
	fi::iso_extract_ctx(c, field, iso, memory, out);
	FI_API_END
}

int fi_iso_extract_field(const float* field, int ndim, const int* sizes, float iso, int memory, fi_mesh** out)
{
	FI_API_BEGIN
	FI_REQUIRE(field && sizes && out, FI_ERR_INVALID, "null argument");
// ... 831 lines not shown
```

field_interpolation_amd/csrc/fi_cg.hip:

```cpp
#include "fi_solver_internal.h"

namespace fi {

namespace {
struct PredKey {
	int    kind, dtype, ndim, gn[3], level, below, mixed, rows_only;
	float  w[8];
	double tol;
	bool operator<(const PredKey& o) const { return std::memcmp(this, &o, sizeof(PredKey)) < 0; }
};
PredKey pred_key(const fi_ctx* c, int kind, double tol)
{
	PredKey k;
	std::memset(&k, 0, sizeof(k));
	k.kind  = kind;
	k.dtype = c->dtype;
	k.ndim  = c->g.ndim;
	for (int d = 0; d < 3; ++d) { k.gn[d] = c->g.gn[d]; }
	k.level = c->level;
	for (const fi_ctx* l = (c->twin && c->twin->coarse ? c->twin->coarse : c->coarse); l; l = l->coarse) { ++k.below; }
	k.mixed     = c->mixed;
	k.rows_only = c->value_rows_only ? 1 : 0;
	const float w[8] = {c->w.data_pos, c->w.data_gradient, c->w.model_0, c->w.model_1, c->w.model_2, c->w.model_3, c->w.model_4,
	                    c->w.gradient_smoothness};
// ... 330 lines not shown
	}
	g.nloc = s;
	g.nown = 1;
	for (int d = 0; d < 3; ++d) { g.nown *= (g.own_hi[d] - g.own_lo[d]); }
	g.own_first = static_cast<int64_t>(g.own_lo[L]) * g.stride[L];
}

int model_reach(const fi_weights& w)
{
	int k = 0;
	if (w.model_1 > 0) { k = 1; }
	if (w.model_2 > 0) { k = 2; }
	if (w.model_3 > 0) { k = 3; }
	if (w.model_4 > 0) { k = 4; }
	return k;
}

void ensure_vectors(fi_ctx* c)
{
	if (c->vectors_ready) { return; }
	const size_t es = elem_size(c);
	const Geom&  g  = c->g;
	const size_t need = es * g.nloc;
	const bool fresh = c->vectors_stale || c->x.bytes < need || c->r.bytes < need || c->p.bytes < need || c->q.bytes < need;
	c->x.alloc(need);
	c->r.alloc(need);
	c->p.alloc(need);
	c->q.alloc(need);
	if (fresh) {
		FI_HIP_TRY(hipMemsetAsync(c->x.p, 0, need, c->stream));
		FI_HIP_TRY(hipMemsetAsync(c->r.p, 0, need, c->stream));
		FI_HIP_TRY(hipMemsetAsync(c->p.p, 0, need, c->stream));
		FI_HIP_TRY(hipMemsetAsync(c->q.p, 0, need, c->stream));
	}
	c->vectors_stale = false;
	int nb = apply_num_partials(c);
	if (nb < 4096) { nb = 4096; }
	if (stencil_cheb_available(c) && nb < stencil_cheb_partials_max(c)) { nb = stencil_cheb_partials_max(c); }
	c->max_blocks = nb;
	c->partial.alloc(sizeof(double) * 4 * nb);
	c->vectors_ready = true;
}

template <typename T>
void load_owned(fi_ctx* c, DevBuf& v, const float* src, int memory)
{
	const Geom& g = c->g;
	if (!src) {
		FI_HIP_TRY(hipMemsetAsync(v.p, 0, sizeof(T) * g.nloc, c->stream));
		return;
	}
	DevBuf tmp;
	const float* dsrc = src;
	if (memory == FI_HOST) {
		tmp.alloc(sizeof(float) * g.nown);
		FI_HIP_TRY(hipMemcpyAsync(tmp.p, src, sizeof(float) * g.nown, hipMemcpyHostToDevice, c->stream));
		dsrc = tmp.as<float>();
	}
	hipLaunchKernelGGL((k_from_float<T>), dim3(blocks_for(g.nown)), dim3(kThreads), 0, c->stream, g.nown, dsrc,
	                   owned<T>(c, v));
	FI_HIP_TRY(hipGetLastError());
	FI_HIP_TRY(hipStreamSynchronize(c->stream));
}

template <typename T>
void store_owned(fi_ctx* c, const DevBuf& v, float* dst, int memory)
{
	const Geom& g = c->g;
	if (!dst) { return; }
	if (memory == FI_DEVICE) {
		hipLaunchKernelGGL((k_to_float<T>), dim3(blocks_for(g.nown)), dim3(kThreads), 0, c->stream, g.nown,
		                   owned<T>(c, v), dst);
		FI_HIP_TRY(hipGetLastError());
		FI_HIP_TRY(hipStreamSynchronize(c->stream));
		return;
	}
	DevBuf tmp;
	tmp.alloc(sizeof(float) * g.nown);
	hipLaunchKernelGGL((k_to_float<T>), dim3(blocks_for(g.nown)), dim3(kThreads), 0, c->stream, g.nown, owned<T>(c, v),
	                   tmp.as<float>());
	FI_HIP_TRY(hipGetLastError());
	FI_HIP_TRY(hipMemcpyAsync(dst, tmp.p, sizeof(float) * g.nown, hipMemcpyDeviceToHost, c->stream));
	FI_HIP_TRY(hipStreamSynchronize(c->stream));
}

void halo_exchange(RankSet& R, DevBuf fi_ctx::*vec, int width)
{
	if (R[0]->nranks == 1) { return; }
	++R[0]->n_halo_exchanges;
	if (R.size() == 1) {
		exchange_halo(R[0], (R[0]->*vec).p, width);
		return;
	}
	for (size_t i = 0; i + 1 < R.size(); ++i) {
		fi_ctx* lo = R[i];
		fi_ctx* hi = R[i + 1];
		const Geom& gl = lo->g;
		const Geom& gh = hi->g;
		const int    L     = gl.ndim - 1;
		const int    H     = width > 0 ? width : lo->reach;
		const size_t es    = elem_size(lo);
		const size_t plane = static_cast<size_t>(gl.stride[L]);
		const size_t bytes = es * plane * H;
		char* lo_base = static_cast<char*>((lo->*vec).p);
		char* hi_base = static_cast<char*>((hi->*vec).p);
		FI_HIP_TRY(hipMemcpyAsync(hi_base + es * plane * (gh.own_lo[L] - H), lo_base + es * plane * (gl.own_hi[L] - H), bytes,
		                          hipMemcpyDeviceToDevice, lo->stream));
		FI_HIP_TRY(hipMemcpyAsync(lo_base + es * plane * gl.own_hi[L], hi_base + es * plane * gh.own_lo[L], bytes,
		                          hipMemcpyDeviceToDevice, lo->stream));
	}
}

bool overlap_possible(const fi_ctx* c)
{
	return c->nranks > 1 && c->march.valid && !c->march.wide && c->march.n_inner > 0 && !c->any_trip && c->generic.ntrip == 0 && c->tile_ts == 0 &&
	       (c->cells.ncell == 0 || cells_fused(c)) && !test_switch("FI_NO_OVERLAP");
}
void exchange_begin(fi_ctx* c, void* v)
{
	if (!c->comm_stream) {
		c->comm_stream = stream_take();
		FI_HIP_TRY(hipEventCreateWithFlags(&c->ev_ready, hipEventDisableTiming));
		FI_HIP_TRY(hipEventCreateWithFlags(&c->ev_halo, hipEventDisableTiming));
	}
	FI_HIP_TRY(hipEventRecord(c->ev_ready, c->stream));
	FI_HIP_TRY(hipStreamWaitEvent(c->comm_stream, c->ev_ready, 0));
	exchange_halo_on(c, v, c->comm_stream);
	FI_HIP_TRY(hipEventRecord(c->ev_halo, c->comm_stream));
}
void exchange_wait(fi_ctx* c) { FI_HIP_TRY(hipStreamWaitEvent(c->stream, c->ev_halo, 0)); }

void apply_exchanged(RankSet& R, DevBuf fi_ctx::*in, DevBuf fi_ctx::*out, double* (*partials_of)(fi_ctx*))
{
	fi_ctx* c0 = R[0];
	if (R.size() == 1 && overlap_possible(c0)) {
		fi_ctx* c = c0;
		double* part = partials_of ? partials_of(c) : nullptr;
		exchange_begin(c, (c->*in).p);
		if (stencil_apply_part(c, (c->*in).p, (c->*out).p, part, 1)) {
			exchange_wait(c);
			stencil_apply_part(c, (c->*in).p, (c->*out).p, part, 2);
			FI_HIP_TRY(hipGetLastError());
			return;
		}
		exchange_wait(c);
		apply_AtA(c, (c->*in).p, (c->*out).p, part);
		return;
	}
	halo_exchange(R, in);
	for (fi_ctx* c : R) { apply_AtA(c, (c->*in).p, (c->*out).p, partials_of ? partials_of(c) : nullptr); }
}

void reset_scalars(RankSet& R, const CgScalars& init)
{
	for (fi_ctx* c : R) {
		FI_HIP_TRY(hipMemcpyAsync(c->scal.p, &init, sizeof(init), hipMemcpyHostToDevice, c->stream));
	}
}

bool timed_out_anywhere(RankSet& R, bool mine)
{
	fi_ctx* c0 = R[0];
	if (!(R.size() == 1 && c0->nranks > 1)) { return mine; }
	double* flag = (c0->scal.as<CgScalars>() + 2)->sums + 3;
	double  v = mine ? 1.0 : 0.0;
	FI_HIP_TRY(hipMemcpyAsync(flag, &v, sizeof(double), hipMemcpyHostToDevice, c0->stream));
// ... 137 lines not shown
			continue;
		}
		if (frame.guard(R)) { break; }
		int burst = kCheckEvery;
		if (c0->level > 0) {
			burst = kCheckEvery / 2;
			if (c0->last_cg_iterations > 0) { burst = looks == 1 ? (c0->last_cg_iterations < 64 ? c0->last_cg_iterations : 64) : 2; }
		}
		for (int k = 0; k < burst; ++k) {
			++issued;
			const bool sample = c0->level == 0 && samples < 8 && (issued & 3) == 1;
			if (sample) { FI_HIP_TRY(hipEventRecord(c0->ev[2 * samples], st)); }
			apply_exchanged(R, &fi_ctx::p, &fi_ctx::q, +[](fi_ctx* c) -> double* { return c->partial.as<double>(); });
			if (sample) {
				FI_HIP_TRY(hipEventRecord(c0->ev[2 * samples + 1], st));
				++samples;
			}
			if (folded) {
				resid_f(c0, c0->partial.as<double>(), nb_apply(c0));
				xp_f(c0, c0->partial.as<double>() + c0->max_blocks, nbf_of(c0));
				continue;
			}
			if (folded_set) {
				reduce_to_slot2(R, 1, nb_apply, zero, +[](fi_ctx* c) -> const double* { return c->partial.as<double>(); });
				for (fi_ctx* c : R) { resid_f(c, (c->scal.as<CgScalars>() + 2)->sums, 1); }
				reduce_to_slot2(R, 2, nbf_of, nbf_of,
				                +[](fi_ctx* c) -> const double* { return c->partial.as<double>() + c->max_blocks; });
				for (fi_ctx* c : R) { xp_f(c, (c->scal.as<CgScalars>() + 2)->sums, 1); }
				continue;
			}
			reduce_phase(R, 1, nb_apply, zero, kPhaseSpmv);
			for (fi_ctx* c : R) {
				const int64_t o = c->g.own_first;
				auto go = [&](auto kernel) {
					hipLaunchKernelGGL(kernel, dim3(nbv(c)), dim3(kThreads), 0, c->stream, c->g.nown, c->scal.as<CgScalars>(),
					                   c->q.as<T>() + o, c->dinv.as<T>() + o, c->r.as<T>() + o, c->partial.as<double>(), nbv(c));
				};
				if (vec_ok(c)) { go(k_cg_resid<T, true>); } else { go(k_cg_resid<T, false>); }
			}
			reduce_phase(R, 2, nbv, nbv, kPhaseUpdate);
			for (fi_ctx* c : R) {
				const int64_t o = c->g.own_first;
				auto go = [&](auto kernel) {
					hipLaunchKernelGGL(kernel, dim3(nbv(c)), dim3(kThreads), 0, c->stream, c->g.nown, c->scal.as<CgScalars>(), issued,
					                   c->r.as<T>() + o, c->dinv.as<T>() + o, c->x.as<T>() + o, c->p.as<T>() + o);
				};
				if (vec_ok(c)) { go(k_cg_xp<T, true>); } else { go(k_cg_xp<T, false>); }
			}
		}
		FI_HIP_TRY(hipGetLastError());
	}
	const CgScalars h = frame.end();
	int used = samples;
	if ((h.iter + 3) / 4 < used) { used = (h.iter + 3) / 4; }
	frame.stats<T>(R, h, used, !c0->verify_residual);
	for (fi_ctx* c : R) {
		c->last_cg_iterations = frame.timed_out ? 0 : h.iter;
		c->cg_count_recalled  = false;
		if (R.size() == 1 && c->level > 0 && !frame.timed_out && (h.done == 1 || h.done == 5)) { remember_iterations(c, 0, tolerance, h.iter); }
	}
	frame.require_ok(h);
}

template <typename T>
void solve_cg_t(fi_ctx* c, const float* guess, int max_iterations, float tol, float* out, int* iterations,
                float* rel_residual, int memory)
{
	ensure_vectors(c);
	c->stats.coarse_iterations = 0;
	RankSet R{c};
	struct Report {
		fi_ctx* c; int* it; float* rel;
		~Report() { if (it) { *it = c->stats.iterations; } if (rel) { *rel = static_cast<float>(c->stats.rel_residual); } }
	} report{c, iterations, rel_residual};
	if (c->guess_native) {
		FI_HIP_TRY(hipMemcpyAsync(owned<T>(c, c->x), c->guess_native, sizeof(T) * c->g.nown, hipMemcpyDeviceToDevice, c->stream));
	} else if (!guess && c->twin && c->twin->coarse) {
		twin_cascade_guess(R);
	} else if (!guess && c->coarse) {
		cascade_guess<T>(R);
	} else {
		load_owned<T>(c, c->x, guess, memory);
	}
	if (test_switch("FI_START_ONLY")) {
		c->stats.iterations = 0;
		store_owned<T>(c, c->x, out, memory);
		return;
	}
	if (c->mg_mode == 1 && (c->coarse || (c->twin && c->twin->coarse))) {
		c->predictable_start = !guess && !c->guess_native;
		cg_run_mg<T>(R, max_iterations, tol);
	} else if (poly_ok(c)) {
		cg_run_poly_or_jacobi<T>(R, max_iterations, tol);
	} else {
		cg_run<T>(R, max_iterations, tol);
	}
	store_owned<T>(c, c->x, out, memory);
}

template <typename T>
__global__ __launch_bounds__(kThreads) void k_tile_rhs(int64_t n, const T* __restrict__ b, const T* __restrict__ ag,
                                                        const T* __restrict__ bg, const T* __restrict__ g,
                                                        T* __restrict__ out)
{
	for (int64_t i = static_cast<int64_t>(blockIdx.x) * kThreads + threadIdx.x; i < n;
	     i += static_cast<int64_t>(gridDim.x) * kThreads) {
		out[i] = b[i] - T(2) * (ag[i] - (bg[i] - T(1e-6f) * g[i]));
	}
}

template <typename T>
void tile_pass_run(RankSet& R, int tile_size)
{
	CgScalars init{};
	reset_scalars(R, init);
	halo_exchange(R, &fi_ctx::x);
	struct Restore {
		RankSet& R;
		std::vector<bool> swapped;
		~Restore()
		{
			for (size_t i = 0; i < R.size(); ++i) {
				fi_ctx* c = R[i];
				c->tile_ts = 0;
				if (swapped[i]) {
					c->atb.swap(c->scratch[21]);
				}
			}
		}
	} restore{R, std::vector<bool>(R.size(), false)};
	for (size_t i = 0; i < R.size(); ++i) {
		fi_ctx* c = R[i];
		DevBuf& rhs = c->scratch[21];
		rhs.alloc(elem_size(c) * c->g.nloc);
		FI_HIP_TRY(hipMemsetAsync(rhs.p, 0, elem_size(c) * c->g.nloc, c->stream));
		apply_AtA(c, c->x.p, c->q.p, nullptr);
		c->tile_ts = tile_size;
		apply_AtA(c, c->x.p, c->r.p, nullptr);
		const int64_t o = c->g.own_first;
		hipLaunchKernelGGL((k_tile_rhs<T>), dim3(stream_blocks(c->g.nown)), dim3(kThreads), 0, c->stream, c->g.nown,
		                   c->atb.as<T>() + o, c->q.as<T>() + o, c->r.as<T>() + o, c->x.as<T>() + o, rhs.as<T>() + o);
		FI_HIP_TRY(hipGetLastError());
		c->atb.swap(rhs);
		restore.swapped[i] = true;
	}
	std::vector<DevBuf*> kept(R.size(), nullptr);
	for (size_t i = 0; i < R.size(); ++i) {
		fi_ctx* c = R[i];
		const fi_weights& w = c->w;
		const bool rows_only = c->generic.nnz > 0 && c->cells.ncell == 0 && c->nranks == 1 && !(w.model_0 > 0) && !(w.model_1 > 0) &&
		                       !(w.model_2 > 0) && !(w.model_3 > 0) && !(w.model_4 > 0) && !(w.gradient_smoothness > 0);
		if (rows_only) {
			DevBuf& g0 = c->scratch[22];
			g0.alloc(elem_size(c) * c->g.nloc);
			FI_HIP_TRY(hipMemcpyAsync(g0.p, c->x.p, elem_size(c) * c->g.nloc, hipMemcpyDeviceToDevice, c->stream));
			kept[i] = &g0;
		}
	}
	cg_run<T>(R, 4000, sizeof(T) == 8 ? 1e-12f : 1e-6f);
	for (size_t i = 0; i < R.size(); ++i) {
		if (kept[i]) { generic_keep_guess_in_empty_tiles(R[i], tile_size, kept[i]->p, R[i]->x.p); }
	}
}

template <typename T>
void tile_pass_t(fi_ctx* c, const float* guess, int tile_size, float* out, int memory)
{
	ensure_vectors(c);
	load_owned<T>(c, c->x, guess, memory);
	RankSet R{c};
	tile_pass_run<T>(R, tile_size);
	store_owned<T>(c, c->x, out, memory);
}

template <typename T>
void jacobi_run(RankSet& R, int sweeps, float weight)
{
	CgScalars init{};
	reset_scalars(R, init);
	for (int s = 0; s < sweeps; ++s) {
// ... 134 lines not shown
```

field_interpolation_amd/csrc/fi_internal.h:

```cpp
#pragma once

#include <hip/hip_runtime.h>

#include <chrono>
#include <cstdint>
#include <cstdio>
#include <cstdlib>
#include <string>
#include <utility>
#include <vector>

#include "../../include/fi_hip.h"

namespace fi {

inline const char* test_switch(const char* name) { return getenv(name); }
#ifdef FI_TIMING_BUILD
inline const char* tuning_switch(const char* name) { return getenv(name); }
#else
inline const char* tuning_switch(const char*) { return nullptr; }
#endif

inline std::chrono::steady_clock::time_point& chain_origin()
{
	static std::chrono::steady_clock::time_point t0;
	return t0;
}
inline void chain_mark(const char* what, int level = -1)
{
	if (!tuning_switch("FI_ASM_CHAIN_TIMES")) { return; }
	if (!what) {
		chain_origin() = std::chrono::steady_clock::now();
		return;
	}
	const double us = std::chrono::duration<double, std::micro>(std::chrono::steady_clock::now() - chain_origin()).count();
	std::fprintf(stderr, "fi_assemble host %8.1f us  %s%s%d\n", us, what, level >= 0 ? " level " : " ", level);
}

void set_error(const char* fmt, ...);

struct Fail {
	int code;
};

#define FI_HIP_TRY(expr)                                                                              \
	do {                                                                                              \
		hipError_t e_ = (expr);                                                                       \
		if (e_ != hipSuccess) {                                                                       \
			::fi::set_error("%s:%d: %s -> %s", __FILE__, __LINE__, #expr, hipGetErrorString(e_));      \
			throw ::fi::Fail{FI_ERR_HIP};                                                             \
		}                                                                                             \
	} while (0)

#define FI_REQUIRE(cond, code, ...)                                                                   \
	do {                                                                                              \
		if (!(cond)) {                                                                                \
			::fi::set_error(__VA_ARGS__);                                                             \
			throw ::fi::Fail{code};                                                                   \
		}                                                                                             \
	} while (0)

void*  pool_take(size_t capacity_wanted, size_t* capacity, size_t* used);
bool   pool_give(void* p, size_t capacity, size_t used);
size_t pool_trim(size_t keep_bytes);
extern thread_local bool pool_quiescent;
extern thread_local hipStream_t alloc_stream;
struct AllocStream {
	hipStream_t was;
	explicit AllocStream(hipStream_t st) : was(alloc_stream) { alloc_stream = st; }
	~AllocStream() { alloc_stream = was; }
	AllocStream(const AllocStream&) = delete;
	AllocStream& operator=(const AllocStream&) = delete;
};
hipStream_t stream_take();
void        stream_give(hipStream_t st, bool drained);
void*       pinned_take(size_t bytes, size_t* capacity);
void        pinned_give(void* p, size_t capacity);

struct DevBuf {
	void*  p     = nullptr;
	size_t bytes = 0;
	size_t cap   = 0;
	DevBuf() = default;
	DevBuf(const DevBuf&) = delete;
	DevBuf& operator=(const DevBuf&) = delete;
	~DevBuf() { release(); }
	void release()
	{
		if (p && !(pool_quiescent && pool_give(p, cap, bytes))) { (void)hipFree(p); }
		p     = nullptr;
		bytes = 0;
		cap   = 0;
	}
	void alloc(size_t nbytes)
	{
// ... 114 lines not shown
	DevBuf      wg_edge, wg_inner, wgp_edge, wgp_inner;
	int         n_edge = 0, n_inner = 0, np_edge = 0, np_inner = 0;
};

struct Tile2Params {
	int nx;
	int nyl;
	int gy;
	int yoff;
	int own_y0, own_y1;
	int tx;
	int tiles_x, tiles_y, ntiles;
};

struct Tile2State {
	bool        valid = false, fused = false;
	Tile2Params P{};
	DevBuf      off;
	DevBuf      pos;
	DevBuf      blk;
	int64_t     nrec = 0;
};

struct GenericRows {
	int64_t ntrip = 0, nrows = 0;
	DevBuf  key;
	DevBuf  val;
	DevBuf  rhs;
	int64_t nnz = 0, ncols = 0;
	DevBuf  csr_ptr, csr_col, csr_val;
	DevBuf  csc_cols, csc_ptr, csc_row, csc_val;
	DevBuf  t;
};

struct Pending {
	int64_t nrows = 0;
	DevBuf  key;
	DevBuf  coef;
	DevBuf  rhs;
};

struct PointBatch {
	long   n = 0;
	DevBuf pos, nrm, pw, val;
	bool   has_nrm = false, has_pw = false, has_val = false;
	float  vw = 0, gw = 0;
	int    vk = 0, gk = 0;
	bool   prior = false;
	DevBuf pw0;
	bool   reweighted = false, had_pw = false;
};

struct RobustState {
	long   n = 0;
	DevBuf omega;
	DevBuf r, keys, sorted, tmp;
	DevBuf rec;
	DevBuf field;
	DevBuf xkeep;
};

struct Comm;
struct NearestIndex;

struct CgScalars {
	double rz, rz_new, pq, rr, bb, tol2, alpha, beta, true_rr;
	double sums[4];
	double rank_max[2 * 16];
	double tscale;
	int    iter, done, max_iter, restarts;
	int    field_min_iter;
	int    field_stopped;
	int    tag, field_ranks;
	double field_tol, field_est, field_kappa;
	unsigned long long dmax_bits, xmax_bits;
	double hist_r[32], hist_s[32], hist_r0;
	double hist_t[32];
};
constexpr int kFieldHist = 32;
constexpr int kFieldRanks = 16;

}

struct fi_ctx {
	int        dtype = FI_F32;
	int        device = 0;
	int        rank = 0, nranks = 1;
	int        n_halo_exchanges = 0;
	int        halo = 0;
	int        min_slab = 0;
	int        reach = 1;
	int        slab_lo = 0, slab_hi = 0;
	bool       slab_fixed = false;
	fi::Geom   g{};
	fi_weights w{};
	bool       model_set = false;
	bool       assembled = false;
	bool       vectors_ready = false;
	bool       vectors_stale = true;
	hipStream_t stream = nullptr;

	std::vector<fi::Pending*> pending;
	std::vector<fi::Pending*> pending_pool;
	std::vector<fi::PointBatch*> batches, batches_pool;
	fi::RobustState robust;
	const void* guess_native = nullptr;
	fi::NearestIndex* nearest = nullptr;

	int        levels_wanted = 0;
	double     coarse_tol = 1e-3;
	fi_ctx*    coarse = nullptr;
	fi_ctx*    finer = nullptr;
	int        level = 0;
	bool       replicated = false;
	int        cc[3] = {0, 0, 0};
	float      pos_shift[3] = {0, 0, 0};
	fi::CellData              cells;
	fi::MarchState            march;
	fi::Tile2State            tile2;
	fi::GenericRows           generic;

	fi::DevBuf atb, diag, dinv;
	fi::DevBuf dinv16;
	fi::DevBuf dinv16s;
	bool       dinv16s_valid = false;
	bool       lumped = false;
	fi::DevBuf dlump;
	hipEvent_t ev_asm0 = nullptr, ev_asm1 = nullptr;
	bool       asm_time_pending = false;
	bool       want_lump = false;
	fi::DevBuf lump;
	bool       data_pinned = false;
	double     mg_safe = 4.0;
	int        mg_terms = 5;
	double     mg_pratio = 30.0;
	int        mg_cheb_degree = 0;
	double     mg_cheb_ratio = 0.0;
	int        mg_kcycle = 0;
	fi::DevBuf kc;
	int        mg_smoother = 1;
	bool       any_trip = false;
	bool       facts_forced = false, forced_trip = false, forced_grad = false;
	bool       value_rows_only = false;
	bool       scaling_ghosts = false;
	bool       defer_scaling_exchange = false;
	fi::DevBuf x, r, p, q;
	fi::DevBuf mg_b, mg_x, mg_r, mg_d;
	double     lambda_max = 0;
	int        poly_terms = 0;
	double     poly_ratio = 10.0;
	double     poly_lambda = 0;
	int        last_mg_iterations = 0;
	double     last_mg_tol = 0;
	bool       predictable_start = false;
	double     last_cg_tol = 0;
	bool       unwatched_pending = false;
	int        unwatched_expected = 0;
	hipEvent_t ev_unwatched = nullptr;
	int        last_cg_iterations = 0;
	double     field_tol = 0;
	bool       pred_recalled[2] = {false, false};
	bool       cg_count_recalled = false;
	int        last_outer_iterations = 0;
	int        mg_mode = 0;
	fi::DevBuf partial;
	fi::DevBuf scal;
	fi::CgScalars* scal_host = nullptr;
	void*      pin[3] = {nullptr, nullptr, nullptr};
	size_t     scal_host_cap = 0;
	size_t     pin_bytes[3] = {0, 0, 0};
	int        max_blocks = 0;

	fi::DevBuf scratch[36];

	bool       bx_dot_wanted = false, bx_dot_done = false;
	bool       tail_ok = false;
	fi::DevBuf tail_dia, tail_map, tail_prog;
	bool       tail_prog_valid = false;
	bool       dia_valid = false;
	int        tail_nlev = 0, tail_nops = 0;
	int        tail_lds_floats = 0;

	fi::Comm*  comm = nullptr;
	hipStream_t comm_stream = nullptr;
	hipStream_t level_stream = nullptr;
	hipEvent_t  ev_level = nullptr;
	hipStream_t level_stream2 = nullptr;
	hipStream_t build_stream = nullptr;
	hipEvent_t  ev_build = nullptr;
	hipEvent_t  ev_level2 = nullptr;
	hipEvent_t  ev_ready = nullptr, ev_halo = nullptr;
	fi::DevBuf group_scal;
	bool       owns_stream = true;
	bool       owns_comm = true;
	int        mixed = 0;
	fi_ctx*    twin = nullptr;
	int        tile_ts = 0;
	int        verify_residual = 1;
	fi_stats   stats{};
	std::vector<hipEvent_t> ev;
	std::vector<hipEvent_t> ev_prec;
	int        prec_budget = 0, prec_taken = 0, prec_chain_launches = 0;
	double     prec_chain_bytes = 0;
};

namespace fi {

size_t elem_size(const fi_ctx* c);

void operator_prepare(fi_ctx* c, bool with_scaling = false, const float* lump_in = nullptr);
void apply_AtA(fi_ctx* c, const void* x, void* y, double* pq_partial);
int  apply_num_partials(const fi_ctx* c);
double apply_algorithmic_bytes(const fi_ctx* c);
void error_map(fi_ctx* c, const void* x, void* out);
void exchange_halo(fi_ctx* c, void* v, int width = 0);
void exchange_halo_on(fi_ctx* c, void* v, hipStream_t stream, int width = 0);
bool comm_ready(const fi_ctx* c);
void operator_finish_ghosts(fi_ctx* c);
void operator_rescale_with_ghosts(fi_ctx* c);
void prepare_safe_scaling(fi_ctx* c);

void stencil_prepare(fi_ctx* c);
int  stencil_partials(const fi_ctx* c);
bool stencil_apply(fi_ctx* c, const void* x, void* y, double* partial);
bool stencil_apply_part(fi_ctx* c, const void* x, void* y, double* partial, int part);

bool cells_fused(const fi_ctx* c);
bool stencil_cheb_available(const fi_ctx* c);
int  stencil_cheb_partials(const fi_ctx* c);
void stencil_cheb_step(fi_ctx* c, const void* z, const void* zprev, const void* r, void* znew, double c1, double c2,
                       double* partial, int part = 0, double zprev_scale = 0.0, double pro_scale = 0.0,
                       const unsigned short* scaling = nullptr,
                       int extend = 0,
                       int fmt = 0,
                       const void* acc = nullptr,
                       const void* dotv = nullptr);
int  stencil_cheb_partials_max(const fi_ctx* c);
bool stencil_cheb_direct(const fi_ctx* c);
bool stencil_full_direct_wanted(const fi_ctx* c);
void stencil_power_step(fi_ctx* c, const void* v, void* vnew, double* partial);
bool stencil_full_epi_available(const fi_ctx* c);
void stencil_full_step(fi_ctx* c, const void* z, const void* zprev, const void* r, bool residual, void* znew, double a,
                       double c1, double c2);
void stencil_lumped_residual(fi_ctx* c, const void* x, const void* b, void* out);

void tile2d_prepare(fi_ctx* c);
int  tile2d_partials(const fi_ctx* c);
bool tile2d_apply(fi_ctx* c, const void* x, void* y, double* partial);
void tile2d_cheb_step(fi_ctx* c, const void* z, const void* zprev, const void* r, void* znew, double c1, double c2, double* partial,
                      double zprev_scale, const unsigned short* scaling);
void tile2d_power_step(fi_ctx* c, const void* v, void* vnew, double* partial);
bool tile2d_full_epi_available(const fi_ctx* c);
void tile2d_full_step(fi_ctx* c, const void* z, const void* zprev, const void* r, bool residual, void* znew, double a, double c1,
                      double c2);

void generic_add_coo(fi_ctx* c, int64_t nrows, int64_t ntrip, const fi_triplet* trip, const float* rhs, int memory);
void generic_add_gradient_linear(fi_ctx* c, long n, const float* pos, const float* nrm, const float* pw, float gw,
                                 float pos_scale = 1.0f, float nrm_scale = 1.0f);
void generic_clear(fi_ctx* c);
void generic_assemble(fi_ctx* c);
int  generic_num_partials(const fi_ctx* c);
void generic_apply(fi_ctx* c, const void* x, void* y, double* partial);
void generic_apply_tile(fi_ctx* c, const void* x, void* y, double* partial, int ts);
void generic_keep_guess_in_empty_tiles(fi_ctx* c, int ts, const void* guess, void* x);
void generic_error_map(fi_ctx* c, const void* x, void* out);

void emit_point_rows(fi_ctx* c, long n, const float* pos, const float* nrm, const float* pw, const float* val,
                     float vw, int vk, float gw, int gk, float pos_scale = 1.0f, float nrm_scale = 1.0f);
void assemble(fi_ctx* c);
void ensure_cell_blocks(fi_ctx* c);
bool stencil_will_fuse(const fi_ctx* c);
void* pinned(fi_ctx* c, int slot, size_t bytes);
// ... 11 lines not shown
```

field_interpolation_amd/csrc/fi_levels.hip:

```cpp
#include "fi_solver_internal.h"
#include "fi_workers.h"

namespace fi {

int plan_levels(const fi_ctx* c, int* first_tail)
{
	const int D = c->g.ndim;
	int n[3] = {c->g.gn[0], c->g.gn[1], c->g.gn[2]};
	std::vector<int> lo(c->nranks), hi(c->nranks);
	for (int r = 0; r < c->nranks; ++r) {
		lo[r] = static_cast<int>(static_cast<int64_t>(r) * n[D - 1] / c->nranks);
		hi[r] = static_cast<int>(static_cast<int64_t>(r + 1) * n[D - 1] / c->nranks);
	}
	int levels = 0, tail = 0;
	const bool allow_tail = c->nranks > 1 && !test_switch("FI_NO_REPLICATED_TAIL");
	for (int l = 1; l <= c->levels_wanted; ++l) {
		bool ok = true;
		for (int d = 0; d < D; ++d) {
			n[d] = (n[d] + 1) / 2;
			ok = ok && n[d] >= 8;
		}
		if (!ok) { break; }
		if (c->nranks > 1 && !tail) {
			bool thick = true;
			for (int r = 0; r < c->nranks; ++r) {
				lo[r] = (lo[r] + 1) / 2;
				hi[r] = (hi[r] + 1) / 2;
				thick = thick && (hi[r] - lo[r]) >= (c->reach > 4 ? c->reach : 4);
			}
			if (!thick) {
				if (!allow_tail) { break; }
				tail = l;
			}
		}
		levels = l;
	}
	if (first_tail) { *first_tail = tail ? tail : levels + 1; }
	return levels;
}

bool holds_value_rows_only(const fi_ctx* src)
{
	for (const PointBatch* b : src->batches) {
		if (b->n > 0 && b->has_nrm && b->gw != 0.0f) { return false; }
	}
	return src->generic.ntrip == 0;
}

void build_levels(fi_ctx* c, fi_ctx* src, hipStream_t build_stream)
{
	if (c->level != 0) { return; }
	if (!src) { src = c; }
	bool wanted = c->levels_wanted > 0;
	if (wanted && c->generic.ntrip > 0) {
		long from_points = 0;
		for (auto* b : src->batches) {
			if (b->has_nrm && b->gk == FI_GRADIENT_LINEAR_INTERPOLATION && b->gw != 0.0f) { from_points += b->n * c->g.ndim; }
		}
		wanted = from_points == c->generic.nrows;
	}
	if (!wanted) {
		if (c->coarse) {
			fi_ctx_destroy(c->coarse);
			c->coarse = nullptr;
		}
		return;
	}
	fi_ctx* fine = c;
	const int D = c->g.ndim;
	std::vector<int> lo(c->nranks), hi(c->nranks);
	for (int r = 0; r < c->nranks; ++r) {
		lo[r] = static_cast<int>(static_cast<int64_t>(r) * c->g.gn[D - 1] / c->nranks);
		hi[r] = static_cast<int>(static_cast<int64_t>(r + 1) * c->g.gn[D - 1] / c->nranks);
	}
	int first_tail = 0;
	const int nlevels = plan_levels(c, &first_tail);
	std::vector<fi_ctx*> built;
	for (int l = 1; l <= nlevels; ++l) {
		const bool tail = l >= first_tail;
		int sizes[3] = {1, 1, 1}, cc[3] = {0, 0, 0};
		float shift[3] = {0, 0, 0};
		for (int d = 0; d < D; ++d) {
			sizes[d] = (fine->g.gn[d] + 1) / 2;
			cc[d] = fine->g.gn[d] % 2 == 0 && (d != D - 1 || c->nranks == 1 || c->reach >= 2 || (tail && fine->replicated)) &&
			        !test_switch("FI_VERTEX_LEVELS");
			shift[d] = 0.5f * (fine->pos_shift[d] - (cc[d] ? 0.5f : 0.0f));
		}
		for (int r = 0; r < c->nranks; ++r) {
			lo[r] = (lo[r] + 1) / 2;
			hi[r] = (hi[r] + 1) / 2;
		}
		int min_slab = sizes[D - 1];
		if (!tail) {
			for (int r = 0; r < c->nranks; ++r) { min_slab = hi[r] - lo[r] < min_slab ? hi[r] - lo[r] : min_slab; }
		}
		const int co_nranks = tail ? 1 : c->nranks;
		fi_ctx* co = fine->coarse;
		if (co && (co->g.gn[0] != sizes[0] || co->g.gn[1] != sizes[1] || co->g.gn[2] != sizes[2] || co->dtype != c->dtype ||
		           co->halo != c->halo || co->cc[0] != cc[0] || co->cc[1] != cc[1] || co->cc[2] != cc[2] || co->nranks != co_nranks)) {
			fi_ctx_destroy(co);
			co = nullptr;
		}
		if (co) {
			for (auto* pb : co->pending) { co->pending_pool.push_back(pb); }
			co->pending.clear();
			generic_clear(co);
		} else {
			co = create_ctx(D, sizes, c->dtype, tail ? 0 : c->rank, co_nranks);
			stream_give(co->stream, true);
			co->stream      = c->stream;
			co->owns_stream = false;
			co->owns_comm   = false;
			co->level       = l;
			co->finer       = fine;
			co->verify_residual = 0;
			co->replicated  = tail;
			if (!tail) {
				co->slab_fixed  = true;
				co->slab_lo     = lo[c->rank];
				co->slab_hi     = hi[c->rank];
			}
			co->halo        = c->halo;
			co->reach       = c->reach;
			for (int d = 0; d < 3; ++d) {
				co->cc[d]        = cc[d];
				co->pos_shift[d] = shift[d];
			}
			compute_geom(co, D, sizes);
			fine->coarse    = co;
		}
		co->min_slab = min_slab;
		co->comm = tail ? nullptr : c->comm;
		co->mg_mode     = c->mg_mode;
		co->mg_smoother = c->mg_smoother;
		co->mg_safe     = c->mg_safe;
		co->mg_terms    = c->mg_terms;
		co->mg_pratio   = c->mg_pratio;
		co->mg_kcycle   = c->mg_kcycle;
		co->mg_cheb_degree = c->mg_cheb_degree;
		co->mg_cheb_ratio  = c->mg_cheb_ratio;
		co->value_rows_only = src->value_rows_only;
		co->any_trip        = src->any_trip;
		co->stream = build_stream ? build_stream : c->stream;
		co->defer_scaling_exchange = build_stream != nullptr;
		const float vol = static_cast<float>(1 << D);
		fi_weights w = fine->w;
		w.model_0 = fine->w.model_0 * std::sqrt(vol);
		w.model_1 = fine->w.model_1 * std::sqrt(vol / 4.0f);
		w.model_2 = fine->w.model_2 * std::sqrt(vol / 16.0f);
		w.model_3 = fine->w.model_3 * std::sqrt(vol / 64.0f);
		w.model_4 = fine->w.model_4 * std::sqrt(vol / 256.0f);
		w.gradient_smoothness = fine->w.gradient_smoothness * std::sqrt(vol / 16.0f);
		co->w = w;
		built.push_back(co);
		fine = co;
	}
	if (fine->coarse) {
		fi_ctx_destroy(fine->coarse);
		fine->coarse = nullptr;
	}
	auto assemble_level = [src](fi_ctx* co) {
		AllocStream alloc_on(co->stream);
		const int   l  = co->level;
		const float ps = 1.0f / static_cast<float>(1 << l), ns = static_cast<float>(1 << l);
		chain_mark("begins:", l);
		for (auto* b : src->batches) {
			const float* nrm = b->has_nrm ? b->nrm.as<float>() : nullptr;
			const float* pw  = b->has_pw ? b->pw.as<float>() : nullptr;
			const float* val = b->has_val ? b->val.as<float>() : nullptr;
			const bool   lin = nrm && b->gk == FI_GRADIENT_LINEAR_INTERPOLATION;
			emit_point_rows(co, b->n, b->pos.as<float>(), nrm, pw, val, b->vw, b->vk, lin ? 0.0f : b->gw * ps,
			                lin ? FI_GRADIENT_CELL_EDGES : b->gk, ps, ns);
			if (lin && b->gw != 0.0f) {
				generic_add_gradient_linear(co, b->n, b->pos.as<float>(), nrm, pw, b->gw * ps, ps, ns);
			}
		}
		chain_mark("rows emitted:", l);
		assemble(co);
		chain_mark("rows assembled:", l);
		generic_assemble(co);
		stencil_prepare(co);
		chain_mark("stencil prepared:", l);
		operator_prepare(co, co->dtype == FI_F32 && co->g.ndim == 3 && co->mg_smoother == 1 && co->value_rows_only && !co->any_trip &&
		                         co->march.valid && !co->march.wide && co->nranks == 1 && !test_switch("FI_MG_FULL_SMOOTHER"));
		co->tail_prog_valid = false;
		co->dia_valid = false;
		chain_mark("operator prepared:", l);
		if (tail_level_supported(co) || stencil_full_direct_wanted(co)) { tail_build_operator(co); }
		chain_mark("done:", l);
		co->assembled = true;
		co->vectors_ready = co->vectors_ready && co->max_blocks >= apply_num_partials(co);
		co->stats.num_unknowns = co->g.nown;
	};
	const bool chains = build_stream != nullptr && built.size() > 1 && !test_switch("FI_SERIAL_LEVEL_CHAINS");
	if (!chains) {
		for (fi_ctx* co : built) { assemble_level(co); }
	} else {
		struct Go {
			hipEvent_t e = nullptr;
			~Go() { if (e) { (void)hipEventDestroy(e); } }
		} go_holder;
		FI_HIP_TRY(hipEventCreateWithFlags(&go_holder.e, hipEventDisableTiming));
		const hipEvent_t go = go_holder.e;
		FI_HIP_TRY(hipEventRecord(go, build_stream));
		std::vector<Worker*> workers;
		std::vector<int>         codes(built.size(), FI_OK);
		std::vector<std::string> msgs(built.size());
		int max_chains = static_cast<int>(built.size());
		if (const char* v = tuning_switch("FI_LEVEL_CHAINS")) { max_chains = std::atoi(v); }
		max_chains = max_chains < 2 ? 2 : max_chains;
		std::vector<size_t> chain_of(built.size(), 0);
		for (size_t i = 1; i < built.size(); ++i) {
			chain_of[i] = 1 + (i - 1) % static_cast<size_t>(max_chains - 1);
			fi_ctx* head = built[chain_of[i]];
			if (!head->build_stream) {
				head->build_stream = stream_take();
				FI_HIP_TRY(hipEventCreateWithFlags(&head->ev_build, hipEventDisableTiming));
			}
			if (chain_of[i] == i) { FI_HIP_TRY(hipStreamWaitEvent(head->build_stream, go, 0)); }
			built[i]->stream = head->build_stream;
		}
		auto guarded = [&](size_t i) {
			try {
				FI_HIP_TRY(hipSetDevice(c->device));
				assemble_level(built[i]);
			} catch (const Fail& f) {
				codes[i] = f.code;
				msgs[i]  = fi_last_error();
			} catch (...) {
				codes[i] = FI_ERR_HIP;
				msgs[i]  = "unexpected exception while assembling a coarser level";
			}
		};
		auto run_chain = [&](size_t head) {
			for (size_t i = head; i < built.size(); ++i) {
				if (chain_of[i] == head) { guarded(i); }
			}
		};
		std::vector<size_t> heads;
		for (size_t i = 1; i < built.size(); ++i) {
			if (chain_of[i] == i) { heads.push_back(i); }
		}
		for (size_t head : heads) {
			Worker* w = nullptr;
			try {
				w = worker_pool().acquire();
				w->run([&run_chain, head]() { run_chain(head); });
			} catch (...) {
				w = nullptr;
			}
			workers.push_back(w);
		}
		guarded(0);
		for (size_t k = 0; k < heads.size(); ++k) {
			Worker* w = workers[k];
			if (w) {
				w->wait();
				worker_pool().release(w);
			} else {
				run_chain(heads[k]);
			}
		}
		for (size_t head : heads) {
			(void)hipEventRecord(built[head]->ev_build, built[head]->build_stream);
			(void)hipStreamWaitEvent(build_stream, built[head]->ev_build, 0);
		}
		for (size_t i = 0; i < built.size(); ++i) {
			if (codes[i] != FI_OK) {
				for (size_t head : heads) { (void)hipStreamSynchronize(built[head]->build_stream); }
				set_error("%s", msgs[i].c_str());
				throw Fail{codes[i]};
			}
		}
	}
	for (fi_ctx* l = c->coarse; l; l = l->coarse) { l->stream = c->stream; }
	{
		std::vector<fi_ctx*> chain;
		for (fi_ctx* l = c->coarse; l; l = l->coarse) { chain.push_back(l); }
		bool ok = true;
		for (size_t k = chain.size(); k-- > 0;) {
			ok = ok && tail_level_supported(chain[k]) && static_cast<int>(chain.size() - k) <= kTailMaxLevels;
			chain[k]->tail_ok = ok;
			chain[k]->tail_prog_valid = false;
		}
	}
	for (fi_ctx* l = c; l; l = l->coarse) { l->lambda_max = 0; }
}

bool lumped_twin_wanted(const fi_ctx* c)
{
	if (test_switch("FI_NO_LUMPED_TWIN") || test_switch("FI_MG_FULL_SMOOTHER") || test_switch("FI_NO_MARCH")) { return false; }
	const fi_weights& w = c->w;
	return c->g.ndim == 3 && c->mg_mode == 1 && c->mg_smoother == 1 && c->levels_wanted > 0 && c->value_rows_only &&
	       c->generic.ntrip == 0 && !c->any_trip && c->g.gn[0] >= 4 && !(w.model_3 > 0 || w.model_4 > 0 || w.gradient_smoothness > 0) &&
	       (w.model_1 > 0 || w.model_2 > 0);
}

__global__ __launch_bounds__(kThreads) void k_lumped_diag(int64_t n, const float* __restrict__ sums, float* __restrict__ dlump,
                                                           float* __restrict__ diag)
{
	for (int64_t i = static_cast<int64_t>(blockIdx.x) * kThreads + threadIdx.x; i < n; i += static_cast<int64_t>(gridDim.x) * kThreads) {
		const float v = sums[i];
		const float f = v > 0.0f ? v : 0.0f;
		dlump[i] = f;
		diag[i]  = f;
	}
}

void twin_assemble_lumped(fi_ctx* c)
{
	fi_ctx* t = c->twin;
	t->stream = c->stream;
	for (auto* pb : t->pending) { t->pending_pool.push_back(pb); }
	t->pending.clear();
	generic_clear(t);
	assemble(t);
	const Geom& g = c->g;
	FI_REQUIRE(c->want_lump && c->lump.p, FI_ERR_STATE, "the lumped replica needs the row sums of the fp64 level's assembly");
	generic_assemble(t);
	stencil_prepare(t);
	if (g.nown == g.nloc && t->nranks == 1 && g.nloc > (1 << 16)) {
		operator_prepare(t, true, c->lump.as<float>());
		return;
	}
	t->dlump.alloc(sizeof(float) * g.nloc);
	if (g.nown != g.nloc) { FI_HIP_TRY(hipMemsetAsync(t->dlump.p, 0, sizeof(float) * g.nloc, c->stream)); }
	hipLaunchKernelGGL(k_lumped_diag, dim3(stream_blocks(g.nown)), dim3(kThreads), 0, c->stream, g.nown,
	                   c->lump.as<float>() + g.own_first, t->dlump.as<float>() + g.own_first, t->diag.as<float>() + g.own_first);
	FI_HIP_TRY(hipGetLastError());
	operator_prepare(t, t->nranks == 1);
}

fi_ctx* twin_prepare(fi_ctx* c)
{
	if (c->level != 0) { return nullptr; }
	if (!(c->mixed && c->dtype == FI_F64)) {
		if (c->twin) {
			fi_ctx_destroy(c->twin);
			c->twin = nullptr;
		}
		return nullptr;
	}
	const int D = c->g.ndim;
	{
		long from_points = 0;
		for (auto* b : c->batches) {
			if (b->has_nrm && b->gk == FI_GRADIENT_LINEAR_INTERPOLATION && b->gw != 0.0f) { from_points += b->n * D; }
		}
		FI_REQUIRE(from_points == c->generic.nrows, FI_ERR_UNSUPPORTED,
		           "mixed precision needs rows that came from points; fi_add_rows_coo rows cannot be replicated");
	}
	int sizes[3] = {c->g.gn[0], c->g.gn[1], c->g.gn[2]};
	fi_ctx* t = c->twin;
	if (t && t->halo != c->halo) {
		fi_ctx_destroy(t);
		t = nullptr;
	}
	if (t) {
		for (auto* pb : t->pending) { t->pending_pool.push_back(pb); }
		t->pending.clear();
		generic_clear(t);
	} else {
		t = create_ctx(D, sizes, FI_F32, c->rank, c->nranks);
		stream_give(t->stream, true);
		t->stream      = c->stream;
		t->owns_stream = false;
		t->owns_comm   = false;
		t->slab_fixed  = true;
		t->slab_lo     = c->slab_lo;
// ... 80 lines not shown
```

field_interpolation_amd/csrc/fi_multigrid.hip:

```cpp
#include "fi_solver_internal.h"
#include "fi_cheb.h"

namespace fi {

template <typename T>
bool cascade_guess(RankSet& R, RankSet* wide)
{
	bool wrote_wide = false;
	std::vector<RankSet> chains;
	{
		RankSet cur = R;
		for (;;) {
			chains.push_back(cur);
			RankSet next;
			for (fi_ctx* c : cur) {
				if (c->coarse) { next.push_back(c->coarse); }
			}
			if (next.size() != cur.size()) { break; }
			cur = next;
		}
	}
	for (auto& lev : chains) {
		for (fi_ctx* c : lev) { ensure_vectors(c); }
	}
	for (fi_ctx* c : chains.back()) { FI_HIP_TRY(hipMemsetAsync(c->x.p, 0, sizeof(T) * c->g.nloc, c->stream)); }
	fi_ctx* root = R[0];
	for (size_t k = chains.size(); k-- > 1;) {
		RankSet& lc = chains[k];
		RankSet& lf = chains[k - 1];
		try {
			for (fi_ctx* l : lc) {
				l->poly_terms = root->poly_terms;
				l->poly_ratio = root->poly_ratio;
				if (const char* e = tuning_switch("FI_COARSE_TERMS")) { l->poly_terms = atoi(e); }
				if (const char* e = tuning_switch("FI_COARSE_RATIO")) { l->poly_ratio = atof(e); }
			}
			const bool mg = root->mg_mode == 1 && lc[0]->coarse && !test_switch("FI_CASCADE_NO_MG");
			for (fi_ctx* l : lc) { l->mg_mode = root->mg_mode; }
			for_each_copy(lc, [&](RankSet& lc) {
			if (poly_ok(lc[0])) {
				cg_run_poly<T>(lc, 0, static_cast<float>(root->coarse_tol));
			} else if (mg) {
				const double floor_tol = sizeof(T) == 4 ? 1e-5 : 0.0;
				const float  ltol = static_cast<float>(root->coarse_tol > floor_tol ? root->coarse_tol : floor_tol);
				int64_t n_level = 1;
				for (int d = 0; d < 3; ++d) { n_level *= lc[0]->g.gn[d]; }
				const int cap_mg = n_level <= (1LL << 22) ? 40 : 8;
				int coarse_it = 0;
				bool finished = false;
				if (lc[0]->value_rows_only) {
					cg_run<T>(lc, 48, ltol);
					coarse_it = lc[0]->stats.iterations;
					finished  = lc[0]->stats.converged != 0;
				}
				if (!finished) {
					for (fi_ctx* l : lc) { l->predictable_start = true; }
					cg_run_mg<T>(lc, cap_mg, ltol);
					coarse_it += lc[0]->stats.iterations;
				}
				for (fi_ctx* l : lc) { l->stats.iterations = coarse_it; }
			} else {
				cg_run<T>(lc, 0, static_cast<float>(root->coarse_tol));
			}
			});
		} catch (const Fail& f) {
			if (f.code != FI_ERR_BREAKDOWN) { throw; }
		}
		root->stats.coarse_iterations += lc[0]->stats.iterations;
		halo_exchange(lc, &fi_ctx::x);
		for (size_t i = 0; i < lf.size(); ++i) {
			const LevelPair L = level_pair(lf[i], lc[i]);
			const bool cubic = L.ndim == 3 && (lf[i]->nranks == 1 || lc[i]->reach >= 2) && !test_switch("FI_LINEAR_START") &&
			                   sizeof(T) * static_cast<size_t>(lc[i]->g.nloc) <= (32u << 20);
			if (cubic && k == 1 && wide && sizeof(T) == 4) {
				launch_prolong_cubic<T, double>(L, lc[i]->x.as<T>(), (*wide)[i]->x.as<double>(), lf[i]->stream);
				wrote_wide = true;
			} else if (cubic) {
				launch_prolong_cubic<T, T>(L, lc[i]->x.as<T>(), lf[i]->x.as<T>(), lf[i]->stream);
			} else {
				launch_prolong<T>(L, lc[i]->x.as<T>(), lf[i]->x.as<T>(), 0, lf[i]->stream);
			}
		}
		FI_HIP_TRY(hipGetLastError());
	}
	return wrote_wide;
}

template <typename T>
__global__ __launch_bounds__(kThreads) void k_cheb_init(int64_t n, const T* __restrict__ b, const T* __restrict__ q,
                                                         const T* __restrict__ dinv, T* __restrict__ r,
                                                         T* __restrict__ d, T* __restrict__ x, T alpha, int zero_x)
{
	for (int64_t i = static_cast<int64_t>(blockIdx.x) * kThreads + threadIdx.x; i < n;
	     i += static_cast<int64_t>(gridDim.x) * kThreads) {
		const T ri = q ? b[i] - q[i] : b[i];
		const T di = alpha * dinv[i] * ri;
		r[i] = ri;
		d[i] = di;
		x[i] = zero_x ? di : x[i] + di;
	}
}

template <typename T>
__global__ __launch_bounds__(kThreads) void k_cheb_iter(int64_t n, const T* __restrict__ q, const T* __restrict__ dinv,
                                                         const T* r_in, T* r, T* d, const T* x_in, T* x, T c1, T c2,
                                                         int store_rd)
{
	for (int64_t i = static_cast<int64_t>(blockIdx.x) * kThreads + threadIdx.x; i < n;
	     i += static_cast<int64_t>(gridDim.x) * kThreads) {
		const T ri = r_in[i] - q[i];
		const T d0 = d[i];
		const T di = c1 * d0 + c2 * dinv[i] * ri;
		const T xi = (x_in == d ? d0 : x_in[i]) + di;
		if (store_rd) {
			r[i] = ri;
			d[i] = di;
		}
		x[i] = xi;
	}
}

template <typename T>
__global__ __launch_bounds__(kThreads) void k_cheb_first(int64_t n, const T* __restrict__ b, const T* __restrict__ dinv,
                                                          T* __restrict__ d, T alpha)
{
	for (int64_t i = static_cast<int64_t>(blockIdx.x) * kThreads + threadIdx.x; i < n;
	     i += static_cast<int64_t>(gridDim.x) * kThreads) {
		d[i] = alpha * dinv[i] * b[i];
	}
}


template <typename T>
__global__ __launch_bounds__(kThreads) void k_sub(int64_t n, const T* __restrict__ b, const T* __restrict__ q,
                                                   T* __restrict__ r)
{
	for (int64_t i = static_cast<int64_t>(blockIdx.x) * kThreads + threadIdx.x; i < n;
	     i += static_cast<int64_t>(gridDim.x) * kThreads) {
		r[i] = b[i] - q[i];
	}
}

template <typename T>
__global__ __launch_bounds__(kThreads) void k_power_step(int64_t n, const T* __restrict__ q, const T* __restrict__ dinv,
                                                          T* __restrict__ v, double* __restrict__ partial)
{
	double acc[1] = {0};
	for (int64_t i = static_cast<int64_t>(blockIdx.x) * kThreads + threadIdx.x; i < n;
	     i += static_cast<int64_t>(gridDim.x) * kThreads) {
		const T w = dinv[i] * q[i];
		v[i] = w;
// ... 1560 lines not shown
```

field_interpolation_amd/csrc/fi_solver_internal.h:

```cpp
#pragma once

#include <chrono>
#include <cmath>
#include <cstdlib>
#include <cstdarg>
#include <cstring>
#include <limits>
#include <map>
#include <mutex>
#include <string>
#include <thread>


#include <type_traits>
#include <vector>

#include "fi_internal.h"
#include "fi_transfer.h"
#include "fi_tail.h"

namespace fi {

using RankSet = std::vector<fi_ctx*>;
using Vec = DevBuf fi_ctx::*;
// ... 403 lines not shown
							const double sj = sc->hist_s[(k - j) % kFieldHist] * f;
							step = sj > step ? sj : step;
							f *= sigma;
						}
					}
					sc->field_est   = kFieldMargin * step * sigma / (1.0 - sigma);
					sc->field_kappa = sc->field_est / (kFieldMargin * rb);
					field_met = sc->field_est <= sc->field_tol && k >= (sc->field_min_iter > 0 ? sc->field_min_iter : kFieldMinIter);
				}
			}
		}
		if (!isfinite(s)) {
			sc->done = 2;
		} else if (field_met || !(s > sc->tol2)) {
			sc->done = 1;
			sc->field_stopped = field_met ? 1 : 0;
		} else if (sc->iter >= sc->max_iter) {
			sc->done = 3;
		}
		break;
	}
	case kMgBeta:
		sc->beta = s / sc->rz;
		sc->rz   = s;
		if (!(s > 0.0) || !isfinite(s)) { sc->done = 2; }
		break;
	case kMgFlex: {
		const double rz_old = sc->beta > 0.0 ? sc->rz / sc->beta : 0.0;
		const double flex = rz_old > 0.0 ? -sc->alpha * s / rz_old : sc->beta;
		if (isfinite(flex)) { sc->beta = flex > 0.0 ? flex : 0.0; }
		break;
	}
	}
}


template <typename T>
__global__ __launch_bounds__(kThreads) void k_cheb_first16(int64_t n, const T* __restrict__ b,
                                                            const unsigned short* __restrict__ dinv16, T* __restrict__ d, T alpha)
{
	for (int64_t i = static_cast<int64_t>(blockIdx.x) * kThreads + threadIdx.x; i < n;
	     i += static_cast<int64_t>(gridDim.x) * kThreads) {
		d[i] = alpha * static_cast<T>(__uint_as_float(static_cast<unsigned int>(dinv16[i]) << 16)) * b[i];
	}
}

template <typename T>
__global__ __launch_bounds__(kThreads) void k_seed(int64_t n, int64_t first, T* __restrict__ v)
{
	for (int64_t i = static_cast<int64_t>(blockIdx.x) * kThreads + threadIdx.x; i < n;
	     i += static_cast<int64_t>(gridDim.x) * kThreads) {
		uint32_t h = static_cast<uint32_t>(first + i) * 2654435761u;
		h ^= h >> 15;
		h *= 2246822519u;
		h ^= h >> 13;
		v[i] = static_cast<T>(static_cast<double>(h & 0xFFFFu) / 65536.0 - 0.5);
	}
}

inline int64_t global_first(const fi_ctx* c)
{
	const Geom& g = c->g;
	const int a = g.ndim - 1;
	int64_t plane = 1;
	for (int d = 0; d < a; ++d) { plane *= g.gn[d]; }
	return plane * (g.off[a] + g.own_lo[a]);
}

inline void residual_rule_stats(fi_stats& s)
{
	s.field_estimate     = -1.0;
	s.field_per_residual = 0.0;
	s.field_rounds       = 0;
	s.stop_residual      = s.rel_residual;
}

}

void compute_geom(fi_ctx* c, int ndim, const int* sizes);
int  model_reach(const fi_weights& w);
void ensure_vectors(fi_ctx* c);
template <typename T> void load_owned(fi_ctx* c, DevBuf& v, const float* src, int memory);
template <typename T> void store_owned(fi_ctx* c, const DevBuf& v, float* dst, int memory);
void halo_exchange(RankSet& R, DevBuf fi_ctx::*vec, int width = 0);
inline const float* field_f32(fi_ctx* c, const float* field, int memory, DevBuf& buf)
{
	const Geom& g = c->g;
	if (field && memory == FI_DEVICE) { return field; }
	if (!field && c->dtype == FI_F32) { return owned<float>(c, c->x); }
	buf.alloc(sizeof(float) * g.nown);
	if (field) {
		FI_HIP_TRY(hipMemcpyAsync(buf.p, field, sizeof(float) * g.nown, hipMemcpyHostToDevice, c->stream));
	} else {
		hipLaunchKernelGGL((k_to_float<double>), dim3(blocks_for(g.nown)), dim3(kThreads), 0, c->stream, g.nown, owned<double>(c, c->x),
		                   buf.as<float>());
		FI_HIP_TRY(hipGetLastError());
	}
	return buf.as<float>();
}
inline void slab_fields(RankSet& R, const float* const* fields, int memory, int want)
{
	for (size_t r = 0; r < R.size(); ++r) {
		fi_ctx*     c = R[r];
		const Geom& g = c->g;
		FI_REQUIRE(fields[r] || c->vectors_ready, FI_ERR_STATE, "no solution yet");
		ensure_vectors(c);
		const size_t es = elem_size(c);
		if (fields[r]) {
			c->dtype == FI_F64 ? load_owned<double>(c, c->q, fields[r], memory) : load_owned<float>(c, c->q, fields[r], memory);
		} else {
			FI_HIP_TRY(hipMemcpyAsync(static_cast<char*>(c->q.p) + es * g.own_first, static_cast<const char*>(c->x.p) + es * g.own_first,
			                          es * g.nown, hipMemcpyDeviceToDevice, c->stream));
		}
	}
	halo_exchange(R, &fi_ctx::q, want);
}
bool overlap_possible(const fi_ctx* c);
void exchange_begin(fi_ctx* c, void* v);
void exchange_wait(fi_ctx* c);
void apply_exchanged(RankSet& R, DevBuf fi_ctx::*in, DevBuf fi_ctx::*out, double* (*partials_of)(fi_ctx*));
void reset_scalars(RankSet& R, const CgScalars& init);
bool timed_out_anywhere(RankSet& R, bool mine);
bool all_ranks_ok(fi_ctx* c, bool mine);
template <typename T> void cg_run(RankSet& R, int max_iterations, float tol);
void remember_iterations(const fi_ctx* c, int kind, double tol, int iterations);
int  recall_iterations(fi_ctx* c, int kind, double tol);
void forget_iterations();
void forget_lambdas();
template <typename T> void solve_cg_t(fi_ctx* c, const float* guess, int max_iterations, float tol, float* out, int* iterations,
                                      float* rel_residual, int memory);
template <typename T> void tile_pass_run(RankSet& R, int tile_size);
template <typename T> void tile_pass_t(fi_ctx* c, const float* guess, int tile_size, float* out, int memory);
template <typename T> void jacobi_run(RankSet& R, int sweeps, float weight);
template <typename T> void jacobi_t(fi_ctx* c, const float* guess, int sweeps, float weight, float* out, int memory);
template <typename T> double true_residual_run(RankSet& R);
template <typename T> double true_residual_t(fi_ctx* c);
template <typename T> void apply_f64_run(RankSet& R, const double* xin, double* yout);
template <typename T> void apply_f64_t(fi_ctx* c, const double* xin, double* yout);
template <typename T> void get_vec_f64_t(fi_ctx* c, const DevBuf& v, double* out);
bool poly_ok(const fi_ctx* c);
void remember_lambda(const fi_ctx* c);
template <typename T> void ensure_poly_vectors(fi_ctx* c);
template <typename T> void estimate_poly_lambda(RankSet& R);
template <typename T> void cg_run_poly(RankSet& R, int max_iterations, float tol);
template <typename T> void cg_run_poly_sr(RankSet& R, int max_iterations, float tol);
template <typename T> void cg_run_poly_or_jacobi(RankSet& R, int max_iterations, float tol);
LevelPair level_pair(const fi_ctx* fine, const fi_ctx* coarse);
template <typename T> void launch_prolong(const LevelPair& L, const T* coarse, T* fine, int mode, hipStream_t st);
template <typename T, typename TO> void launch_prolong_cubic(const LevelPair& L, const T* coarse, TO* fine, hipStream_t st);
template <typename T> void launch_restrict(const LevelPair& L, const T* fine, T* coarse, hipStream_t st, T* tmp = nullptr, int f_local_planes = 0);
template <typename T> bool cascade_guess(RankSet& R, RankSet* wide = nullptr);
void twin_cascade_guess(RankSet& R);
template <typename T> void cg_run_mg(RankSet& R, int max_iterations, float tol);
template <typename T> void mg_alloc(fi_ctx* c);
int  plan_levels(const fi_ctx* c, int* first_tail);
bool holds_value_rows_only(const fi_ctx* src);
void build_levels(fi_ctx* c, fi_ctx* src = nullptr, hipStream_t build_stream = nullptr);
fi_ctx* twin_prepare(fi_ctx* c);
void twin_assemble(fi_ctx* c, hipStream_t build_stream);
void twin_assemble_lumped(fi_ctx* c);
bool lumped_twin_wanted(const fi_ctx* c);
void twin_finish(fi_ctx* c);
void build_twin(fi_ctx* c);
fi_ctx* create_ctx(int ndim, const int* sizes, int dtype, int rank, int nranks);
void check_ctx(const fi_ctx* c);
void check_assembled(const fi_ctx* c);
void bind_device(const fi_ctx* c);

namespace {
bool replicated_copies(const RankSet& R) { return R.size() > 1 && R[0]->nranks == 1; }
template <typename Fn>
void for_each_copy(RankSet& R, Fn fn)
{
	if (replicated_copies(R)) {
		for (fi_ctx* c : R) {
			RankSet one{c};
			fn(one);
		}
	} else {
		fn(R);
	}
}


template <typename CountFn>
void mg_reduce(RankSet& R, CountFn count_of, int phase)
{
	if (R.size() == 1 && R[0]->nranks == 1) {
		fi_ctx* c = R[0];
		hipLaunchKernelGGL(k_mg_logic, dim3(1), dim3(kThreads), 0, c->stream, c->scal.as<CgScalars>(), c->partial.as<double>(),
		                   count_of(c), phase);
		return;
	}
	reduce_phase(R, 1, count_of, count_of, -1);
	for (fi_ctx* c : R) {
		hipLaunchKernelGGL(k_mg_logic, dim3(1), dim3(kThreads), 0, c->stream, c->scal.as<CgScalars>(),
		                   static_cast<const double*>(nullptr), 0, phase);
	}
}

inline void top_up_events(std::vector<hipEvent_t>& ev, int count)
{
	while (static_cast<int>(ev.size()) < count) {
		hipEvent_t e;
		FI_HIP_TRY(hipEventCreate(&e));
		ev.push_back(e);
	}
}

struct SolveFrame {
	fi_ctx* const     c0;
	const hipStream_t st;
	int               max_iterations;
	double            tolerance;
	EventPair         timer;
	double limit_s   = 600.0;
	bool   timed_out = false;
	float  ms        = 0;
	std::chrono::steady_clock::time_point wall0 = std::chrono::steady_clock::now();

	SolveFrame(RankSet& R, int max_it, float tol) : c0(R[0]), st(R[0]->stream), max_iterations(max_it)
	{
		if (max_iterations <= 0) {
			const int64_t dflt = 2 * static_cast<int64_t>(c0->g.gn[0]) * c0->g.gn[1] * c0->g.gn[2];
			max_iterations = dflt > std::numeric_limits<int>::max() ? std::numeric_limits<int>::max() : static_cast<int>(dflt);
		}
		tolerance = tol > 0 ? static_cast<double>(tol) : static_cast<double>(std::numeric_limits<float>::epsilon());
		if (const char* env = getenv("FI_SOLVE_TIMEOUT_S")) { limit_s = atof(env); }
	}
	void begin()
	{
		FI_HIP_TRY(hipEventRecord(timer.e0, st));
		wall0 = std::chrono::steady_clock::now();
	}
	const CgScalars& look(const CgScalars* slot)
	{
		FI_HIP_TRY(hipMemcpyAsync(c0->scal_host, slot, sizeof(CgScalars), hipMemcpyDeviceToHost, st));
		FI_HIP_TRY(hipStreamSynchronize(st));
		return *c0->scal_host;
	}
	bool guard(RankSet& R)
	{
		timed_out = timed_out_anywhere(R, std::chrono::duration<double>(std::chrono::steady_clock::now() - wall0).count() > limit_s);
		return timed_out;
	}
	CgScalars end()
	{
		FI_HIP_TRY(hipEventRecord(timer.e1, st));
		FI_HIP_TRY(hipEventSynchronize(timer.e1));
		FI_HIP_TRY(hipEventElapsedTime(&ms, timer.e0, timer.e1));
		return *c0->scal_host;
	}
	template <typename T>
	void stats(RankSet& R, const CgScalars& h, int used, bool done1_ok)
	{
		double sum_ms = 0;
		for (int k = 0; k < used; ++k) {
			float t = 0;
			FI_HIP_TRY(hipEventElapsedTime(&t, c0->ev[2 * k], c0->ev[2 * k + 1]));
			sum_ms += t;
		}
		for (fi_ctx* c : R) {
			c->stats.spmv_samples = used;
			c->stats.spmv_ms_avg  = used ? sum_ms / used : 0.0;
			c->stats.spmv_bytes   = apply_algorithmic_bytes(c);
			c->stats.prec_samples = 0;
			c->stats.prec_ms_avg  = 0.0;
			c->stats.prec_bytes   = 0.0;
			c->stats.operator_applies = h.iter + 1 + h.restarts;
			c->stats.solve_ms     = ms;
			c->stats.iterations   = h.iter;
			c->stats.converged    = (!timed_out && (h.done == 4 || h.done == 5 || (h.done == 1 && done1_ok))) ? 1 : 0;
			c->stats.rel_residual = h.bb > 0 ? std::sqrt(h.rr / h.bb) : 0.0;
			c->stats.restarts     = h.restarts;
			c->stats.verified_residual = (h.restarts > 0 && h.bb > 0) ? std::sqrt(h.true_rr / h.bb) : -1.0;
			residual_rule_stats(c->stats);
			if (h.done == 4) {
				FI_HIP_TRY(hipMemsetAsync(c->x.p, 0, sizeof(T) * c->g.nloc, c->stream));
			}
		}
	}
	void require_ok(const CgScalars& h, const char* breakdown = nullptr) const
	{
		if (breakdown) { FI_REQUIRE(h.done != 2, FI_ERR_BREAKDOWN, "%s", breakdown); }
		FI_REQUIRE(h.done != 2, FI_ERR_BREAKDOWN, "CG breakdown: non-finite or non-positive curvature (p.AtA p = %g)", h.pq);
		FI_REQUIRE(!timed_out, FI_ERR_TIMEOUT, "solve stopped by the wall-clock guard (FI_SOLVE_TIMEOUT_S = %g s) after %d iterations, "
		           "relative residual %g", limit_s, h.iter, h.bb > 0 ? std::sqrt(h.rr / h.bb) : 0.0);
	}
};

}

}

#define FI_API_BEGIN try {
#define FI_API_END                                                   \
	}                                                                \
	catch (const fi::Fail& f) { return f.code; }                     \
	catch (const std::exception& e)                                  \
	{                                                                \
		fi::set_error("exception: %s", e.what());                    \
		return FI_ERR_INVALID;                                       \
	}                                                                \
	catch (...)                                                      \
	{                                                                \
		fi::set_error("unknown exception");                          \
		return FI_ERR_INVALID;                                       \
	}                                                                \
	return FI_OK;
```

include/fi_hip.h:

```cpp
#ifndef FI_HIP_H
#define FI_HIP_H

#ifdef __cplusplus
extern "C" {
#endif

#define FI_OK 0
#define FI_ERR_INVALID 1
#define FI_ERR_HIP 2
#define FI_ERR_STATE 3
#define FI_ERR_COMM 4
#define FI_ERR_UNSUPPORTED 5
#define FI_ERR_BREAKDOWN 6
#define FI_ERR_TIMEOUT 7

#define FI_HOST 0
#define FI_DEVICE 1

#define FI_F32 0
#define FI_F64 1

#define FI_MAX_DIM 3

#define FI_SAMPLE_LINEAR 0
// ... 77 lines not shown
int fi_comm_unique_id(void* out128);
int fi_comm_init(fi_ctx* ctx, const void* unique_id128);
int fi_comm_info(const fi_ctx* ctx, long out[7]);
int fi_comm_init_host(fi_ctx* ctx, const char* name, int create);

int fi_set_model(fi_ctx* ctx, const fi_weights* w);

int fi_add_points(fi_ctx* ctx, long n, const float* positions, const float* normals, const float* point_weights,
                  const float* values, float value_weight, int value_kernel, float gradient_weight,
                  int gradient_kernel, int memory);

int fi_add_border_prior(fi_ctx* ctx, float weight);

int fi_add_rows_coo(fi_ctx* ctx, long nrows, long ntriplets, const fi_triplet* triplets, const float* rhs,
                    int memory);

int fi_assemble(fi_ctx* ctx);

int fi_clear_points(fi_ctx* ctx);

int fi_solve_cg(fi_ctx* ctx, const float* guess, int max_iterations, float tol, float* out, int* iterations,
                float* rel_residual, int memory);

#define FI_OPT_VERIFY_RESIDUAL 1
#define FI_OPT_LEVELS 2
#define FI_OPT_COARSE_TOLERANCE 3
#define FI_OPT_MULTIGRID 4
#define FI_OPT_MIXED_PRECISION 5
#define FI_OPT_POLY_TERMS 6
#define FI_OPT_POLY_RATIO 7
#define FI_OPT_MG_SMOOTHER 8
#define FI_OPT_MG_SAFE_FACTOR 9
#define FI_OPT_MG_TERMS 10
#define FI_OPT_MG_RATIO 11
#define FI_OPT_FIELD_TOLERANCE 12
#define FI_OPT_MG_KCYCLE 13
#define FI_OPT_MG_CHEB_DEGREE 14
#define FI_OPT_MG_CHEB_RATIO 15
int fi_set_option(fi_ctx* ctx, int option, double value);

int fi_jacobi(fi_ctx* ctx, const float* guess, int num_iterations, float weight, float* out, int memory);

int fi_tile_pass(fi_ctx* ctx, const float* guess, int tile_size, float* out, int memory);

int fi_error_map(fi_ctx* ctx, const float* solution, float* out, int memory);

#define FI_LOSS_HUBER 0
#define FI_LOSS_CAUCHY 1
#define FI_LOSS_TUKEY 2

typedef struct fi_robust_options {
	int   loss;
	float tuning;
	float scale;
	int   rounds;
	float weight_tolerance;
} fi_robust_options;

typedef struct fi_robust_stats {
	int    rounds;
	int    iterations;
	float  scale;
	float  max_weight_change;
	long   points_used;
	long   points_zeroed;
	double reweight_ms;
} fi_robust_stats;

int fi_point_count(const fi_ctx* ctx, long* n);
int fi_point_residuals(fi_ctx* ctx, const float* field, float* residuals, int memory);
int fi_robust_reweight(fi_ctx* ctx, const float* field, const fi_robust_options* options, float* omega, float* scale, int memory);
int fi_reset_point_weights(fi_ctx* ctx);
int fi_solve_robust(fi_ctx* ctx, const float* guess, const fi_robust_options* options, int max_iterations, float tol, float* out,
                    float* omega, fi_robust_stats* stats, int memory);

int fi_get_solution_f64(fi_ctx* ctx, double* out);

int fi_true_residual(fi_ctx* ctx, double* rel_residual);

int fi_apply_AtA_f64(fi_ctx* ctx, const double* x, double* y);
int fi_get_Atb_f64(fi_ctx* ctx, double* out);
int fi_get_diag_f64(fi_ctx* ctx, double* out);
int fi_get_stats(const fi_ctx* ctx, fi_stats* out);
int fi_memory_pool(long long keep_bytes, long long* cached_bytes);
int fi_time_apply(fi_ctx* ctx, int reps, double* ms_per_launch);

typedef struct fi_group fi_group;
typedef struct fi_mesh fi_mesh;
typedef struct fi_points fi_points;
typedef struct fi_surface fi_surface;
int     fi_group_create(fi_group** out, int ndim, const int* sizes, int dtype, int nranks);
int     fi_group_destroy(fi_group* g);
int     fi_group_size(const fi_group* g);
fi_ctx* fi_group_rank(fi_group* g, int rank);
int     fi_group_assemble(fi_group* g);
int     fi_group_solve_cg(fi_group* g, const float* guess, int max_iterations, float tol, float* out, int* iterations,
                          float* rel_residual);
int     fi_group_apply_AtA_f64(fi_group* g, const double* x, double* y);
int     fi_group_true_residual(fi_group* g, double* rel_residual);
int     fi_group_get_solution_f64(fi_group* g, double* out);
int     fi_group_tile_pass(fi_group* g, const float* guess, int tile_size, float* out);
int     fi_group_error_map(fi_group* g, const float* solution, float* out);
int     fi_group_iso_extract(fi_group* g, const float* whole_or_null, float iso, fi_mesh** out);
int     fi_group_sample(fi_group* g, const float* whole_or_null, long n, const float* positions, int mode, float fill,
                        float* values, float* gradients);

int fi_upscale_field(const float* small_field, int ndim, const int* small_sizes, const int* large_sizes,
                     float* out, int memory);

int fi_iso_extract(fi_ctx* ctx, const float* field, float iso, int memory, fi_mesh** out);
int fi_iso_extract_field(const float* field, int ndim, const int* sizes, float iso, int memory, fi_mesh** out);

int fi_dual_contour(fi_ctx* ctx, const float* field, const float* gradients, float iso, int memory, fi_mesh** out);
int fi_dual_contour_field(const float* field, const float* gradients, int ndim, const int* sizes, float iso, int memory,
                          fi_mesh** out);

int fi_mesh_info(const fi_mesh* m, long* num_vertices, long* num_primitives, int* vertices_per_primitive);
int fi_mesh_copy(const fi_mesh* m, float* vertices, float* normals, int* indices, long long* keys, int memory);
int fi_mesh_destroy(fi_mesh* m);

typedef struct fi_mesh_part {
	long long vertices, primitives, edges, boundary, irregular;
	double    size, enclosed;
	float     lo[3], hi[3];
} fi_mesh_part;
int fi_mesh_create(fi_mesh** out, int ndim, long num_vertices, const float* vertices, const float* normals,
                   const long long* keys, long num_primitives, const int* indices, int memory);
int fi_mesh_parts(const fi_mesh* m, long* num_parts, int* vertex_labels, int* primitive_labels, int memory);
int fi_mesh_measure(const fi_mesh* m, long capacity, fi_mesh_part* parts, long* num_parts);
int fi_mesh_select(const fi_mesh* m, long num_parts, const unsigned char* keep, fi_mesh** out);

#define FI_SIMPLIFY_QUADRIC 0
#define FI_SIMPLIFY_MEAN    1
int fi_mesh_simplify(const fi_mesh* m, float cell, const float* origin, int placement, int* vertex_map, int memory,
                     fi_mesh** out);

#define FI_SMOOTH_BOUNDARY_FIXED 0
#define FI_SMOOTH_BOUNDARY_SLIDE 1
#define FI_SMOOTH_BOUNDARY_FREE  2
#define FI_SMOOTH_NORMALS_RECOMPUTE 0
#define FI_SMOOTH_NORMALS_KEEP      1
typedef struct fi_smooth_options {
	int   iterations;
	float lambda, mu;
	int   boundary;
	float max_move;
	int   normals;
} fi_smooth_options;
int fi_mesh_smooth(const fi_mesh* m, const fi_smooth_options* opt, fi_mesh** out);
int fi_mesh_normals(const fi_mesh* m, fi_mesh** out);

#define FI_SAMPLE_NORMALS_FACE   0
#define FI_SAMPLE_NORMALS_VERTEX 1
typedef struct fi_deviation {
	long long queries, counted, beyond, invalid, at;
	double    max, mean, rms;
	float     where[3];
} fi_deviation;
int fi_mesh_sample(const fi_mesh* m, long n, unsigned long long seed, int normals_mode, float* positions, float* normals,
                   long long* primitives, int memory);
int fi_mesh_deviation(const fi_mesh* a, fi_surface* b, long samples, unsigned long long seed, float max_distance,
                      fi_deviation* of_samples, fi_deviation* of_vertices, float* vertex_distances, int memory);

#define FI_REGISTER_PLANE 0
#define FI_REGISTER_POINT 1
#define FI_LOSS_NONE (-1)
// ... 161 lines not shown
```

Baseline: 1.858 billion.

## Defer coarse multigrid level assembly joins into the solve and fuse solution store

When assembly settings match the previous call on a single-rank context, coarse-level builds are left running on a worker thread and build streams. fi_assemble now returns early, and each level is joined on demand during the multigrid solve, coarsest first. The solution conversion and copy-out are also enqueued before the end-of-solve stream sync, which removes a second synchronisation. This overlaps host-side level construction with the start of the solve, at the cost of much more complex error handling and state tracking across API calls.

```diff
diff --git a/field_interpolation_amd/_capi.py b/field_interpolation_amd/_capi.py
--- a/field_interpolation_amd/_capi.py
+++ b/field_interpolation_amd/_capi.py
@@ -15,7 +15,7 @@
     "fi_slab_range", "fi_slab_point_range", "fi_slab_partition", "fi_halo_width", "fi_comm_unique_id", "fi_comm_init", "fi_comm_init_host", "fi_comm_info", "fi_comm_self_test", "fi_set_model", "fi_add_points", "fi_add_border_prior",
     "fi_add_rows_coo", "fi_assemble", "fi_clear_points", "fi_set_option", "fi_solve_cg", "fi_jacobi", "fi_tile_pass", "fi_error_map",
     "fi_get_solution_f64", "fi_true_residual", "fi_apply_AtA_f64", "fi_get_Atb_f64", "fi_get_diag_f64",
-    "fi_get_stats", "fi_memory_pool", "fi_time_apply", "fi_upscale_field",
+    "fi_get_stats", "fi_levels_pending", "fi_memory_pool", "fi_time_apply", "fi_upscale_field",
     "fi_group_create", "fi_group_destroy", "fi_group_size", "fi_group_rank", "fi_group_assemble",
     "fi_group_solve_cg", "fi_group_apply_AtA_f64", "fi_group_true_residual", "fi_group_get_solution_f64", "fi_group_tile_pass", "fi_group_error_map",
     "fi_group_iso_extract", "fi_iso_extract", "fi_iso_extract_field", "fi_mesh_info", "fi_mesh_copy", "fi_mesh_destroy",
@@ -190,6 +190,7 @@
     L.fi_get_Atb_f64.argtypes = [vp, dp]
     L.fi_get_diag_f64.argtypes = [vp, dp]
     L.fi_get_stats.argtypes = [vp, C.POINTER(FiStats)]
+    L.fi_levels_pending.argtypes = [vp, C.POINTER(C.c_int)]
     L.fi_time_apply.argtypes = [vp, C.c_int, dp]
     L.fi_memory_pool.argtypes = [C.c_longlong, C.POINTER(C.c_longlong)]
     L.fi_upscale_field.argtypes = [fp, C.c_int, ip, ip, fp, C.c_int]
diff --git a/field_interpolation_amd/api.py b/field_interpolation_amd/api.py
--- a/field_interpolation_amd/api.py
+++ b/field_interpolation_amd/api.py
@@ -1760,6 +1760,11 @@
         check(_capi.lib().fi_get_stats(self._h, C.byref(s)))
         return {name: getattr(s, name) for name, _ in FiStats._fields_}
 
+    def levels_pending(self):
+        n = C.c_int(0)
+        check(_capi.lib().fi_levels_pending(self._h, C.byref(n)))
+        return n.value
+
     def time_apply(self, reps=20):
         self._ready()
         ms = C.c_double(0)
diff --git a/field_interpolation_amd/csrc/fi_capi.hip b/field_interpolation_amd/csrc/fi_capi.hip
--- a/field_interpolation_amd/csrc/fi_capi.hip
+++ b/field_interpolation_amd/csrc/fi_capi.hip
@@ -110,7 +110,14 @@
 void check_assembled(const fi_ctx* c)
 {
 	check_ctx(c);
+	join_levels(const_cast<fi_ctx*>(c));
 	FI_REQUIRE(c->assembled, FI_ERR_STATE, "fi_assemble has not been called");
+}
+
+void check_ctx_idle(fi_ctx* c)
+{
+	check_ctx(c);
+	join_levels(c);
 }
 
 void bind_device(const fi_ctx* c) { FI_HIP_TRY(hipSetDevice(c->device)); }
@@ -191,6 +198,7 @@
 {
 	if (!c) { return FI_OK; }
 	(void)hipSetDevice(c->device);
+	fi::abandon_levels(c);
 	bool drained = true;
 	for (hipStream_t st : {c->stream, c->level_stream, c->level_stream2, c->build_stream, c->comm_stream}) {
 		if (st && hipStreamSynchronize(st) != hipSuccess) { drained = false; }
@@ -213,10 +221,9 @@
 	fi::stream_give(c->level_stream, drained);
 	if (c->ev_level) { (void)hipEventDestroy(c->ev_level); }
 	fi::stream_give(c->level_stream2, drained);
-	if (c->build_stream) {
-		fi::stream_give(c->build_stream, drained);
-		(void)hipEventDestroy(c->ev_build);
-	}
+	if (c->build_stream) { fi::stream_give(c->build_stream, drained); }
+	if (c->ev_build) { (void)hipEventDestroy(c->ev_build); }
+	if (c->join.ev_main) { (void)hipEventDestroy(c->join.ev_main); }
 	if (c->ev_level2) { (void)hipEventDestroy(c->ev_level2); }
 	if (c->comm_stream) {
 		fi::stream_give(c->comm_stream, drained);
@@ -303,7 +310,7 @@
 int fi_set_model(fi_ctx* c, const fi_weights* w)
 {
 	FI_API_BEGIN
-	fi::check_ctx(c);
+	fi::check_ctx_idle(c);
 	FI_REQUIRE(w != nullptr, FI_ERR_INVALID, "weights is null");
 	c->w         = *w;
 	c->model_set = true;
@@ -320,7 +327,7 @@
                   int memory)
 {
 	FI_API_BEGIN
-	fi::check_ctx(c);
+	fi::check_ctx_idle(c);
 	fi::bind_device(c);
 	FI_REQUIRE(n >= 0, FI_ERR_INVALID, "negative point count");
 	if (n == 0) { return FI_OK; }
@@ -404,7 +411,7 @@
 int fi_add_border_prior(fi_ctx* c, float weight)
 {
 	FI_API_BEGIN
-	fi::check_ctx(c);
+	fi::check_ctx_idle(c);
 	fi::bind_device(c);
 	if (weight == 0.0f) { return FI_OK; }
 	FI_REQUIRE(c->nranks == 1, FI_ERR_UNSUPPORTED, "fi_add_border_prior on a slab context: a rank sees only its own points");
@@ -427,7 +434,7 @@
 int fi_add_rows_coo(fi_ctx* c, long nrows, long ntriplets, const fi_triplet* triplets, const float* rhs, int memory)
 {
 	FI_API_BEGIN
-	fi::check_ctx(c);
+	fi::check_ctx_idle(c);
 	fi::bind_device(c);
 	FI_REQUIRE(nrows >= 0 && ntriplets >= 0, FI_ERR_INVALID, "negative count");
 	fi::check_memory(memory);
@@ -441,7 +448,7 @@
 int fi_clear_points(fi_ctx* c)
 {
 	FI_API_BEGIN
-	fi::check_ctx(c);
+	fi::check_ctx_idle(c);
 	for (auto* pb : c->pending) { c->pending_pool.push_back(pb); }
 	c->pending.clear();
 	for (auto* b : c->batches) { c->batches_pool.push_back(b); }
@@ -467,8 +474,11 @@
 int fi_assemble(fi_ctx* c)
 {
 	FI_API_BEGIN
-	fi::check_ctx(c);
-	fi::bind_device(c);
+	fi::check_ctx_idle(c);
+	fi::bind_device(c);
+	const bool in_group = c->facts_forced;
+	const bool had_settings = c->join.have_settings;
+	c->join.have_settings = false;
 	fi::finish_assemble_timing(c);
 	if (!c->ev_asm0) {
 		FI_HIP_TRY(hipEventCreate(&c->ev_asm0));
@@ -529,6 +539,7 @@
 	const bool mixed64 = c->mixed && c->dtype == FI_F64;
 	c->want_lump = mixed64 && fi::lumped_twin_wanted(c);
 	const bool beside = (c->levels_wanted > 0 || mixed64) && !c->any_trip && !fi::test_switch("FI_SERIAL_LEVELS");
+	bool settings_ok = false;
 	if (beside && mixed64) {
 		const int keep = c->levels_wanted;
 		c->levels_wanted = 0;
@@ -542,8 +553,11 @@
 		}
 		FI_HIP_TRY(hipEventRecord(c->ev_level, c->stream));
 		FI_HIP_TRY(hipStreamWaitEvent(c->level_stream, c->ev_level, 0));
-		int         helper_code = FI_OK;
-		std::string helper_msg;
+		fi::LevelJoin& J = c->join;
+		int&         helper_code = J.code[0];
+		std::string& helper_msg  = J.msg[0];
+		helper_code = FI_OK;
+		helper_msg.clear();
 		if (mixed64) {
 			fi::twin_prepare(c);
 			if (!c->level_stream2) {
@@ -552,7 +566,33 @@
 			}
 			FI_HIP_TRY(hipStreamWaitEvent(c->level_stream2, c->ev_level, 0));
 		}
-		auto guarded = [&](auto&& work, int* code, std::string* msg) {
+		const bool lumped = mixed64 && c->twin && c->twin->lumped;
+		fi::LevelSettings settings_now;
+		{
+			fi::LevelSettings& s = settings_now;
+			s.dtype = c->dtype; s.mixed = c->mixed; s.levels_wanted = c->levels_wanted; s.mg_mode = c->mg_mode;
+			s.mg_smoother = c->mg_smoother; s.mg_terms = c->mg_terms; s.mg_kcycle = c->mg_kcycle; s.mg_cheb_degree = c->mg_cheb_degree;
+			s.halo = c->halo; s.reach = c->reach;
+			for (int d = 0; d < 3; ++d) { s.gn[d] = c->g.gn[d]; }
+			s.mg_safe = c->mg_safe; s.mg_pratio = c->mg_pratio; s.mg_cheb_ratio = c->mg_cheb_ratio;
+			s.value_rows_only = c->value_rows_only; s.lumped = lumped; s.w = c->w;
+			for (const fi_ctx* l = mixed64 ? c->twin : c; l && l->coarse; l = l->coarse) { s.num_levels += 1; }
+			int first_tail = 0;
+			if (fi::plan_levels(c, &first_tail) != s.num_levels) { s.num_levels = -1; }
+		}
+		const bool lazy = had_settings && settings_now.same(J.settings) && settings_now.num_levels > 0 && c->nranks == 1 && !in_group &&
+		                  !fi::test_switch("FI_EAGER_LEVELS");
+		J.slot  = mixed64 ? 1 : 0;
+		J.first = nullptr;
+		J.levels_left = 0;
+		if (lazy) {
+			J.setup.arm();
+			if (!J.ev_main) { FI_HIP_TRY(hipEventCreateWithFlags(&J.ev_main, hipEventDisableTiming)); }
+		}
+		J.timing_parties.store(lazy ? 2 : 0);
+		fi_ctx* const cc = c;
+		auto guarded = [cc](auto&& work, int* code, std::string* msg) {
+			fi_ctx* const c = cc;
 			try {
 				FI_HIP_TRY(hipSetDevice(c->device));
 				fi::AllocStream none(nullptr);
@@ -565,21 +605,32 @@
 				*msg  = "unexpected exception while building the coarser levels";
 			}
 		};
-		const bool lumped = mixed64 && c->twin && c->twin->lumped;
-		auto build = [&]() {
+		auto build = [cc, guarded, lumped, mixed64, lazy]() {
+			fi_ctx* const c = cc;
 			guarded([&]() {
 				if (lumped) {
 				} else if (mixed64) {
 					fi::twin_assemble(c, c->level_stream);
 				} else {
-					fi::build_levels(c, nullptr, c->level_stream);
+					fi::build_levels(c, nullptr, c->level_stream, lazy);
 				}
-			}, &helper_code, &helper_msg);
+			}, &c->join.code[0], &c->join.msg[0]);
+			if (lazy && !mixed64) {
+				fi::close_levels(c, c, c->join.code[0], c->join.msg[0]);
+				fi::close_assemble_timing(c);
+			}
 		};
-		int         helper2_code = FI_OK;
-		std::string helper2_msg;
-		auto build2 = [&]() {
-			guarded([&]() { fi::build_levels(c->twin, c, c->level_stream2); }, &helper2_code, &helper2_msg);
+		int&         helper2_code = J.code[1];
+		std::string& helper2_msg  = J.msg[1];
+		helper2_code = FI_OK;
+		helper2_msg.clear();
+		auto build2 = [cc, guarded, lazy]() {
+			fi_ctx* const c = cc;
+			guarded([&]() { fi::build_levels(c->twin, c, c->level_stream2, lazy); }, &c->join.code[1], &c->join.msg[1]);
+			if (lazy) {
+				fi::close_levels(c, c->twin, c->join.code[1], c->join.msg[1]);
+				fi::close_assemble_timing(c);
+			}
 		};
 		fi::Worker *helper = nullptr, *helper2 = nullptr;
 		try {
@@ -624,28 +675,53 @@
 				fi::set_error("unexpected exception while building the lumped replica");
 			}
 		}
+		fi::Worker* in_flight = nullptr;
 		if (helper) {
-			helper->wait();
-			fi::worker_pool().release(helper);
+			if (lazy && !mixed64 && main_code == FI_OK) {
+				in_flight = helper;
+			} else {
+				helper->wait();
+				fi::worker_pool().release(helper);
+			}
 		} else if (main_code == FI_OK && !lumped) {
 			build();
 		}
 		if (mixed64) {
 			if (helper2) {
-				helper2->wait();
-				fi::worker_pool().release(helper2);
+				if (lazy && main_code == FI_OK && helper_code == FI_OK) {
+					in_flight = helper2;
+				} else {
+					helper2->wait();
+					fi::worker_pool().release(helper2);
+				}
 			} else if (main_code == FI_OK) {
 				build2();
 			}
-			if (helper_code == FI_OK && helper2_code != FI_OK) {
-				helper_code = helper2_code;
-				helper_msg  = helper2_msg;
+		}
+		if (in_flight) {
+			std::string setup_msg;
+			if (J.setup.wait(&setup_msg) != FI_OK) {
+				in_flight->wait();
+				fi::worker_pool().release(in_flight);
+				in_flight = nullptr;
 			}
+		}
+		if (in_flight) {
+			J.worker  = in_flight;
+			J.pending = true;
+		}
+		if (mixed64 && !in_flight && helper_code == FI_OK && helper2_code != FI_OK) {
+			helper_code = helper2_code;
+			helper_msg  = helper2_msg;
 		}
 		fi::chain_mark("helpers joined");
 		fi_ctx* const first_built = mixed64 ? c->twin : c->coarse;
-		for (fi_ctx* l = first_built; l; l = l->coarse) { l->stream = c->stream; }
-		const bool mine_ok = main_code == FI_OK && helper_code == FI_OK;
+		if (!lazy) {
+			for (fi_ctx* l = first_built; l; l = l->coarse) { l->stream = c->stream; }
+		} else if (mixed64) {
+			c->twin->stream = c->stream;
+		}
+		const bool mine_ok = main_code == FI_OK && ((in_flight && !mixed64) || helper_code == FI_OK);
 		bool peers_ok = true;
 		try {
 			peers_ok = fi::all_ranks_ok(c, mine_ok);
@@ -664,7 +740,7 @@
 			fi::set_error("fi_assemble: another rank failed while assembling its slab");
 			throw fi::Fail{FI_ERR_COMM};
 		}
-		if (fi::tuning_switch("FI_ASM_CHAIN_TIMES")) {
+		if (fi::tuning_switch("FI_ASM_CHAIN_TIMES") && !lazy) {
 			hipEvent_t a = nullptr, b = nullptr, d = nullptr;
 			FI_HIP_TRY(hipEventCreate(&a));
 			FI_HIP_TRY(hipEventCreate(&b));
@@ -684,15 +760,31 @@
 			(void)hipEventDestroy(b);
 			(void)hipEventDestroy(d);
 		}
-		FI_HIP_TRY(hipEventRecord(c->ev_level, c->level_stream));
-		FI_HIP_TRY(hipStreamWaitEvent(c->stream, c->ev_level, 0));
+		if (!lazy || (mixed64 && !lumped)) {
+			FI_HIP_TRY(hipEventRecord(c->ev_level, c->level_stream));
+			FI_HIP_TRY(hipStreamWaitEvent(c->stream, c->ev_level, 0));
+		}
 		if (mixed64) {
-			FI_HIP_TRY(hipEventRecord(c->ev_level2, c->level_stream2));
-			FI_HIP_TRY(hipStreamWaitEvent(c->stream, c->ev_level2, 0));
+			if (!lazy) {
+				FI_HIP_TRY(hipEventRecord(c->ev_level2, c->level_stream2));
+				FI_HIP_TRY(hipStreamWaitEvent(c->stream, c->ev_level2, 0));
+			}
 			fi::twin_finish(c);
 		}
 		fi::operator_finish_ghosts(c);
-		for (fi_ctx* l = first_built; l; l = l->coarse) { fi::operator_finish_ghosts(l); }
+		if (!lazy) {
+			for (fi_ctx* l = first_built; l; l = l->coarse) { fi::operator_finish_ghosts(l); }
+		} else {
+			if (mixed64) { fi::operator_finish_ghosts(c->twin); }
+			if (!in_flight) {
+				J.pending = true;
+				fi::join_levels(c);
+			}
+		}
+		settings_ok = true;
+		c->join.settings = settings_now;
+		c->join.settings.num_levels = 0;
+		for (const fi_ctx* l = first_built && mixed64 ? first_built : c; l && l->coarse; l = l->coarse) { c->join.settings.num_levels += 1; }
 	} else {
 	fi::AllocStream alloc_on(c->stream);
 	fi::assemble(c);
@@ -712,7 +804,13 @@
 		fi::build_levels(c);
 		fi::build_twin(c);
 	}
-	FI_HIP_TRY(hipEventRecord(e1, c->stream));
+	if (c->join.pending) {
+		FI_HIP_TRY(hipEventRecord(c->join.ev_main, c->stream));
+		fi::close_assemble_timing(c);
+	} else {
+		FI_HIP_TRY(hipEventRecord(e1, c->stream));
+	}
+	c->join.have_settings = settings_ok;
 	fi::chain_mark("fi_assemble returns");
 	c->asm_time_pending   = true;
 	c->stats.assemble_ms  = 0.0;
@@ -730,7 +828,8 @@
                 float* rel_residual, int memory)
 {
 	FI_API_BEGIN
-	fi::check_assembled(c);
+	fi::check_ctx(c);
+	if (guess || c->guess_native || !c->assembled) { fi::check_assembled(c); }
 	fi::bind_device(c);
 	fi::check_memory(memory);
 	fi::AllocStream alloc_on(c->stream);
@@ -745,7 +844,7 @@
 int fi_set_option(fi_ctx* c, int option, double value)
 {
 	FI_API_BEGIN
-	fi::check_ctx(c);
+	fi::check_ctx_idle(c);
 	switch (option) {
 	case FI_OPT_VERIFY_RESIDUAL: c->verify_residual = value != 0.0; break;
 	case FI_OPT_LEVELS:
@@ -860,7 +959,7 @@
 int fi_point_residuals(fi_ctx* c, const float* field, float* residuals, int memory)
 {
 	FI_API_BEGIN
-	fi::check_ctx(c);
+	fi::check_ctx_idle(c);
 	fi::bind_device(c);
 	fi::check_memory(memory);
 	fi::robust_residuals(c, field, residuals, memory);
@@ -870,7 +969,7 @@
 int fi_robust_reweight(fi_ctx* c, const float* field, const fi_robust_options* options, float* omega, float* scale, int memory)
 {
 	FI_API_BEGIN
-	fi::check_ctx(c);
+	fi::check_ctx_idle(c);
 	fi::bind_device(c);
 	FI_REQUIRE(options != nullptr, FI_ERR_INVALID, "options is null");
 	fi::check_memory(memory);
@@ -882,7 +981,7 @@
 int fi_reset_point_weights(fi_ctx* c)
 {
 	FI_API_BEGIN
-	fi::check_ctx(c);
+	fi::check_ctx_idle(c);
 	fi::bind_device(c);
 	fi::robust_reset(c);
 	FI_API_END
@@ -1018,6 +1117,7 @@
 	FI_API_BEGIN
 	fi::check_ctx(c);
 	FI_REQUIRE(out != nullptr, FI_ERR_INVALID, "null output");
+	fi::join_levels(const_cast<fi_ctx*>(c));
 	fi::finish_assemble_timing(const_cast<fi_ctx*>(c));
 	*out = c->stats;
 	out->coarse_unconverged = 0;
@@ -1030,6 +1130,15 @@
 		if (!met) { out->coarse_unconverged += 1; }
 		out->coarse_iterations += (met ? was->iter : l->unwatched_expected) - l->unwatched_expected;
 	}
+	FI_API_END
+}
+
+int fi_levels_pending(const fi_ctx* c, int* count)
+{
+	FI_API_BEGIN
+	fi::check_ctx(c);
+	FI_REQUIRE(count != nullptr, FI_ERR_INVALID, "null output");
+	*count = c->join.pending ? c->join.levels_left : 0;
 	FI_API_END
 }
 
diff --git a/field_interpolation_amd/csrc/fi_cg.hip b/field_interpolation_amd/csrc/fi_cg.hip
--- a/field_interpolation_amd/csrc/fi_cg.hip
+++ b/field_interpolation_amd/csrc/fi_cg.hip
@@ -436,6 +436,25 @@
 	FI_HIP_TRY(hipGetLastError());
 	FI_HIP_TRY(hipMemcpyAsync(dst, tmp.p, sizeof(float) * g.nown, hipMemcpyDeviceToHost, c->stream));
 	FI_HIP_TRY(hipStreamSynchronize(c->stream));
+}
+
+void store_solution_async(fi_ctx* c)
+{
+	const Geom& g = c->g;
+	float* dst = c->store_dst;
+	if (c->store_memory != FI_DEVICE) {
+		c->store_tmp.alloc(sizeof(float) * g.nown);
+		dst = c->store_tmp.as<float>();
+	}
+	if (c->dtype == FI_F64) {
+		hipLaunchKernelGGL((k_to_float<double>), dim3(blocks_for(g.nown)), dim3(kThreads), 0, c->stream, g.nown, owned<double>(c, c->x), dst);
+	} else {
+		hipLaunchKernelGGL((k_to_float<float>), dim3(blocks_for(g.nown)), dim3(kThreads), 0, c->stream, g.nown, owned<float>(c, c->x), dst);
+	}
+	FI_HIP_TRY(hipGetLastError());
+	if (c->store_memory != FI_DEVICE) {
+		FI_HIP_TRY(hipMemcpyAsync(c->store_dst, c->store_tmp.p, sizeof(float) * g.nown, hipMemcpyDeviceToHost, c->stream));
+	}
 }
 
 void halo_exchange(RankSet& R, DevBuf fi_ctx::*vec, int width)
@@ -739,20 +758,34 @@
 	} else {
 		load_owned<T>(c, c->x, guess, memory);
 	}
+	join_levels(c);
 	if (test_switch("FI_START_ONLY")) {
 		c->stats.iterations = 0;
 		store_owned<T>(c, c->x, out, memory);
 		return;
 	}
-	if (c->mg_mode == 1 && (c->coarse || (c->twin && c->twin->coarse))) {
-		c->predictable_start = !guess && !c->guess_native;
-		cg_run_mg<T>(R, max_iterations, tol);
-	} else if (poly_ok(c)) {
-		cg_run_poly_or_jacobi<T>(R, max_iterations, tol);
-	} else {
-		cg_run<T>(R, max_iterations, tol);
-	}
-	store_owned<T>(c, c->x, out, memory);
+	struct Store {
+		fi_ctx* c;
+		Store(fi_ctx* ctx, float* dst, int memory) : c(ctx)
+		{
+			c->store_dst      = dst;
+			c->store_memory   = memory;
+			c->store_enqueued = false;
+		}
+		~Store() { c->store_dst = nullptr; }
+	};
+	{
+		Store store(c, out, memory);
+		if (c->mg_mode == 1 && (c->coarse || (c->twin && c->twin->coarse))) {
+			c->predictable_start = !guess && !c->guess_native;
+			cg_run_mg<T>(R, max_iterations, tol);
+		} else if (poly_ok(c)) {
+			cg_run_poly_or_jacobi<T>(R, max_iterations, tol);
+		} else {
+			cg_run<T>(R, max_iterations, tol);
+		}
+	}
+	if (!c->store_enqueued) { store_owned<T>(c, c->x, out, memory); }
 }
 
 template <typename T>
diff --git a/field_interpolation_amd/csrc/fi_internal.h b/field_interpolation_amd/csrc/fi_internal.h
--- a/field_interpolation_amd/csrc/fi_internal.h
+++ b/field_interpolation_amd/csrc/fi_internal.h
@@ -2,6 +2,7 @@
 
 #include <hip/hip_runtime.h>
 
+#include <atomic>
 #include <chrono>
 #include <cstdint>
 #include <cstdio>
@@ -11,6 +12,7 @@
 #include <vector>
 
 #include "../../include/fi_hip.h"
+#include "fi_latch.h"
 
 namespace fi {
 
@@ -291,6 +293,41 @@
 
 }
 
+namespace fi {
+class Worker;
+struct LevelSettings {
+	int        dtype = 0, mixed = 0, levels_wanted = 0, mg_mode = 0, mg_smoother = 0, mg_terms = 0, mg_kcycle = 0, mg_cheb_degree = 0;
+	int        halo = 0, reach = 0, gn[3] = {0, 0, 0}, num_levels = 0;
+	double     mg_safe = 0, mg_pratio = 0, mg_cheb_ratio = 0;
+	bool       value_rows_only = false, lumped = false;
+	fi_weights w{};
+	bool same(const LevelSettings& o) const
+	{
+		return dtype == o.dtype && mixed == o.mixed && levels_wanted == o.levels_wanted && mg_mode == o.mg_mode &&
+		       mg_smoother == o.mg_smoother && mg_terms == o.mg_terms && mg_kcycle == o.mg_kcycle && mg_cheb_degree == o.mg_cheb_degree &&
+		       halo == o.halo && reach == o.reach && gn[0] == o.gn[0] && gn[1] == o.gn[1] && gn[2] == o.gn[2] && num_levels == o.num_levels &&
+		       mg_safe == o.mg_safe && mg_pratio == o.mg_pratio && mg_cheb_ratio == o.mg_cheb_ratio && value_rows_only == o.value_rows_only &&
+		       lumped == o.lumped && w.data_pos == o.w.data_pos && w.data_gradient == o.w.data_gradient && w.model_0 == o.w.model_0 &&
+		       w.model_1 == o.w.model_1 && w.model_2 == o.w.model_2 && w.model_3 == o.w.model_3 && w.model_4 == o.w.model_4 &&
+		       w.gradient_smoothness == o.w.gradient_smoothness && w.value_kernel == o.w.value_kernel && w.gradient_kernel == o.w.gradient_kernel;
+	}
+};
+struct LevelJoin {
+	Latch         setup;
+	Worker*       worker = nullptr;
+	int           code[2] = {0, 0};
+	std::string   msg[2];
+	int           slot = 0;
+	bool          pending = false;
+	fi_ctx*       first = nullptr;
+	int           levels_left = 0;
+	std::atomic<int> timing_parties{0};
+	hipEvent_t    ev_main = nullptr;
+	bool          have_settings = false;
+	LevelSettings settings;
+};
+}
+
 struct fi_ctx {
 	int        dtype = FI_F32;
 	int        device = 0;
@@ -354,6 +391,10 @@
 	bool       scaling_ghosts = false;
 	bool       defer_scaling_exchange = false;
 	fi::DevBuf x, r, p, q;
+	float*     store_dst = nullptr;
+	int        store_memory = 0;
+	bool       store_enqueued = false;
+	fi::DevBuf store_tmp;
 	fi::DevBuf mg_b, mg_x, mg_r, mg_d;
 	double     lambda_max = 0;
 	int        poly_terms = 0;
@@ -397,6 +438,11 @@
 	hipStream_t level_stream2 = nullptr;
 	hipStream_t build_stream = nullptr;
 	hipEvent_t  ev_build = nullptr;
+	fi::Latch   built;
+	bool        join_pending = false;
+	hipStream_t join_stream = nullptr;
+	fi_ctx*     join_root = nullptr;
+	fi::LevelJoin join;
 	hipEvent_t  ev_level2 = nullptr;
 	hipEvent_t  ev_ready = nullptr, ev_halo = nullptr;
 	fi::DevBuf group_scal;
diff --git a/field_interpolation_amd/csrc/fi_latch.h b/field_interpolation_amd/csrc/fi_latch.h
--- /dev/null
+++ b/field_interpolation_amd/csrc/fi_latch.h
@@ -0,0 +1,52 @@
+#pragma once
+
+#include <condition_variable>
+#include <mutex>
+#include <string>
+#include <utility>
+
+namespace fi {
+
+class Latch {
+public:
+	void arm()
+	{
+		std::lock_guard<std::mutex> g(m_);
+		set_  = false;
+		code_ = 0;
+		msg_.clear();
+	}
+	bool set(int code = 0, std::string msg = std::string())
+	{
+		{
+			std::lock_guard<std::mutex> g(m_);
+			if (set_) { return false; }
+			set_  = true;
+			code_ = code;
+			msg_  = std::move(msg);
+		}
+		cv_.notify_all();
+		return true;
+	}
+	int wait(std::string* msg = nullptr)
+	{
+		std::unique_lock<std::mutex> g(m_);
+		cv_.wait(g, [this]() { return set_; });
+		if (msg) { *msg = msg_; }
+		return code_;
+	}
+	bool is_set()
+	{
+		std::lock_guard<std::mutex> g(m_);
+		return set_;
+	}
+
+private:
+	std::mutex              m_;
+	std::condition_variable cv_;
+	bool                    set_  = true;
+	int                     code_ = 0;
+	std::string             msg_;
+};
+
+}
diff --git a/field_interpolation_amd/csrc/fi_levels.hip b/field_interpolation_amd/csrc/fi_levels.hip
--- a/field_interpolation_amd/csrc/fi_levels.hip
+++ b/field_interpolation_amd/csrc/fi_levels.hip
@@ -47,7 +47,7 @@
 	return src->generic.ntrip == 0;
 }
 
-void build_levels(fi_ctx* c, fi_ctx* src, hipStream_t build_stream)
+void build_levels(fi_ctx* c, fi_ctx* src, hipStream_t build_stream, bool lazy)
 {
 	if (c->level != 0) { return; }
 	if (!src) { src = c; }
@@ -143,6 +143,7 @@
 		co->any_trip        = src->any_trip;
 		co->stream = build_stream ? build_stream : c->stream;
 		co->defer_scaling_exchange = build_stream != nullptr;
+		co->join_pending = false;
 		const float vol = static_cast<float>(1 << D);
 		fi_weights w = fine->w;
 		w.model_0 = fine->w.model_0 * std::sqrt(vol);
@@ -192,9 +193,58 @@
 		co->vectors_ready = co->vectors_ready && co->max_blocks >= apply_num_partials(co);
 		co->stats.num_unknowns = co->g.nown;
 	};
+	auto settle = [&]() {
+		std::vector<fi_ctx*> chain;
+		for (fi_ctx* l = c->coarse; l; l = l->coarse) { chain.push_back(l); }
+		bool ok = true;
+		for (size_t k = chain.size(); k-- > 0;) {
+			ok = ok && tail_level_supported(chain[k]) && static_cast<int>(chain.size() - k) <= kTailMaxLevels;
+			chain[k]->tail_ok = ok;
+			chain[k]->tail_prog_valid = false;
+		}
+		for (fi_ctx* l = c; l; l = l->coarse) { l->lambda_max = 0; }
+	};
 	const bool chains = build_stream != nullptr && built.size() > 1 && !test_switch("FI_SERIAL_LEVEL_CHAINS");
+	auto hand_over = [&](fi_ctx* co, int code, std::string msg) {
+		if (!lazy) { return; }
+		if (code == FI_OK && hipEventRecord(co->ev_build, co->stream) != hipSuccess) {
+			code = FI_ERR_HIP;
+			msg  = "hipEventRecord failed behind a coarser level's assembly";
+		}
+		co->built.set(code, std::move(msg));
+	};
+	auto arm = [&]() {
+		if (!lazy) { return; }
+		FI_REQUIRE(build_stream != nullptr && src->nranks == 1, FI_ERR_STATE, "lazy levels need a build stream and an undivided lattice");
+		for (fi_ctx* co : built) {
+			if (!co->ev_build) { FI_HIP_TRY(hipEventCreateWithFlags(&co->ev_build, hipEventDisableTiming)); }
+		}
+		settle();
+		for (fi_ctx* co : built) {
+			co->built.arm();
+			co->join_pending = true;
+			co->join_stream  = src->stream;
+			co->join_root    = src;
+		}
+		src->join.first       = built.empty() ? nullptr : built[0];
+		src->join.levels_left = static_cast<int>(built.size());
+		src->join.setup.set(FI_OK);
+	};
 	if (!chains) {
-		for (fi_ctx* co : built) { assemble_level(co); }
+		arm();
+		for (fi_ctx* co : built) {
+			if (!lazy) {
+				assemble_level(co);
+				continue;
+			}
+			try {
+				assemble_level(co);
+			} catch (const Fail& f) {
+				hand_over(co, f.code, fi_last_error());
+				throw;
+			}
+			hand_over(co, FI_OK, std::string());
+		}
 	} else {
 		struct Go {
 			hipEvent_t e = nullptr;
@@ -220,6 +270,7 @@
 			if (chain_of[i] == i) { FI_HIP_TRY(hipStreamWaitEvent(head->build_stream, go, 0)); }
 			built[i]->stream = head->build_stream;
 		}
+		arm();
 		auto guarded = [&](size_t i) {
 			try {
 				FI_HIP_TRY(hipSetDevice(c->device));
@@ -231,6 +282,7 @@
 				codes[i] = FI_ERR_HIP;
 				msgs[i]  = "unexpected exception while assembling a coarser level";
 			}
+			hand_over(built[i], codes[i], msgs[i]);
 		};
 		auto run_chain = [&](size_t head) {
 			for (size_t i = head; i < built.size(); ++i) {
@@ -262,6 +314,7 @@
 			}
 		}
 		for (size_t head : heads) {
+			if (lazy) { break; }
 			(void)hipEventRecord(built[head]->ev_build, built[head]->build_stream);
 			(void)hipStreamWaitEvent(build_stream, built[head]->ev_build, 0);
 		}
@@ -273,18 +326,97 @@
 			}
 		}
 	}
+	if (lazy) { return; }
 	for (fi_ctx* l = c->coarse; l; l = l->coarse) { l->stream = c->stream; }
-	{
-		std::vector<fi_ctx*> chain;
-		for (fi_ctx* l = c->coarse; l; l = l->coarse) { chain.push_back(l); }
-		bool ok = true;
-		for (size_t k = chain.size(); k-- > 0;) {
-			ok = ok && tail_level_supported(chain[k]) && static_cast<int>(chain.size() - k) <= kTailMaxLevels;
-			chain[k]->tail_ok = ok;
-			chain[k]->tail_prog_valid = false;
-		}
-	}
-	for (fi_ctx* l = c; l; l = l->coarse) { l->lambda_max = 0; }
+	settle();
+}
+
+void finish_level(fi_ctx* l)
+{
+	if (!l->join_pending) { return; }
+	std::string msg;
+	chain_mark("awaited:", l->level);
+	const int code = l->built.wait(&msg);
+	chain_mark("joined:", l->level);
+	l->join_pending = false;
+	l->stream = l->join_stream;
+	fi_ctx* root = l->join_root;
+	LevelJoin& J = root->join;
+	J.levels_left -= 1;
+	if (code != FI_OK) {
+		root->assembled = false;
+		J.have_settings = false;
+		set_error("%s", msg.c_str());
+		throw Fail{code};
+	}
+	operator_finish_ghosts(l);
+	FI_HIP_TRY(hipStreamWaitEvent(l->join_stream, l->ev_build, 0));
+}
+
+void close_assemble_timing(fi_ctx* root)
+{
+	LevelJoin& J = root->join;
+	if (J.timing_parties.fetch_sub(1) != 1) { return; }
+	const hipStream_t ts = root->level_stream;
+	for (fi_ctx* k = J.first; k; k = k->coarse) { (void)hipStreamWaitEvent(ts, k->ev_build, 0); }
+	(void)hipStreamWaitEvent(ts, J.ev_main, 0);
+	(void)hipEventRecord(root->ev_asm1, ts);
+}
+
+void join_levels(fi_ctx* c)
+{
+	LevelJoin& J = c->join;
+	if (!J.pending) { return; }
+	J.pending = false;
+	if (J.worker) {
+		J.worker->wait();
+		worker_pool().release(J.worker);
+		J.worker = nullptr;
+	}
+	int         code = J.code[J.slot];
+	std::string msg  = J.msg[J.slot];
+	std::vector<fi_ctx*> levels;
+	for (fi_ctx* l = J.first; l; l = l->coarse) { levels.push_back(l); }
+	for (size_t k = levels.size(); k-- > 0;) {
+		try {
+			finish_level(levels[k]);
+		} catch (const Fail& f) {
+			if (code == FI_OK) {
+				code = f.code;
+				msg  = fi_last_error();
+			}
+		}
+	}
+	if (code != FI_OK) {
+		for (fi_ctx* l : levels) {
+			if (l->build_stream) { (void)hipStreamSynchronize(l->build_stream); }
+		}
+		if (c->level_stream) { (void)hipStreamSynchronize(c->level_stream); }
+		if (c->level_stream2) { (void)hipStreamSynchronize(c->level_stream2); }
+		c->assembled       = false;
+		J.have_settings    = false;
+		c->asm_time_pending = false;
+		set_error("%s", msg.c_str());
+		throw Fail{code};
+	}
+}
+
+void abandon_levels(fi_ctx* c)
+{
+	LevelJoin& J = c->join;
+	if (J.worker) {
+		J.worker->wait();
+		worker_pool().release(J.worker);
+		J.worker = nullptr;
+	}
+	J.pending = false;
+}
+
+void close_levels(fi_ctx* root, fi_ctx* top, int code, const std::string& msg)
+{
+	const bool armed = !root->join.setup.set(code, msg);
+	if (code == FI_OK || !armed) { return; }
+	for (fi_ctx* l = top ? top->coarse : nullptr; l; l = l->coarse) { l->built.set(code, msg); }
 }
 
 bool lumped_twin_wanted(const fi_ctx* c)
diff --git a/field_interpolation_amd/csrc/fi_multigrid.hip b/field_interpolation_amd/csrc/fi_multigrid.hip
--- a/field_interpolation_amd/csrc/fi_multigrid.hip
+++ b/field_interpolation_amd/csrc/fi_multigrid.hip
@@ -20,9 +20,13 @@
 			cur = next;
 		}
 	}
-	for (auto& lev : chains) {
-		for (fi_ctx* c : lev) { ensure_vectors(c); }
-	}
+	auto ready = [](RankSet& lev) {
+		for (fi_ctx* c : lev) {
+			finish_level(c);
+			ensure_vectors(c);
+		}
+	};
+	ready(chains.back());
 	for (fi_ctx* c : chains.back()) { FI_HIP_TRY(hipMemsetAsync(c->x.p, 0, sizeof(T) * c->g.nloc, c->stream)); }
 	fi_ctx* root = R[0];
 	for (size_t k = chains.size(); k-- > 1;) {
@@ -67,6 +71,7 @@
 			if (f.code != FI_ERR_BREAKDOWN) { throw; }
 		}
 		root->stats.coarse_iterations += lc[0]->stats.iterations;
+		ready(lf);
 		halo_exchange(lc, &fi_ctx::x);
 		for (size_t i = 0; i < lf.size(); ++i) {
 			const LevelPair L = level_pair(lf[i], lc[i]);
diff --git a/field_interpolation_amd/csrc/fi_solver_internal.h b/field_interpolation_amd/csrc/fi_solver_internal.h
--- a/field_interpolation_amd/csrc/fi_solver_internal.h
+++ b/field_interpolation_amd/csrc/fi_solver_internal.h
@@ -509,6 +509,7 @@
 void ensure_vectors(fi_ctx* c);
 template <typename T> void load_owned(fi_ctx* c, DevBuf& v, const float* src, int memory);
 template <typename T> void store_owned(fi_ctx* c, const DevBuf& v, float* dst, int memory);
+void store_solution_async(fi_ctx* c);
 void halo_exchange(RankSet& R, DevBuf fi_ctx::*vec, int width = 0);
 inline const float* field_f32(fi_ctx* c, const float* field, int memory, DevBuf& buf)
 {
@@ -582,7 +583,12 @@
 template <typename T> void mg_alloc(fi_ctx* c);
 int  plan_levels(const fi_ctx* c, int* first_tail);
 bool holds_value_rows_only(const fi_ctx* src);
-void build_levels(fi_ctx* c, fi_ctx* src = nullptr, hipStream_t build_stream = nullptr);
+void build_levels(fi_ctx* c, fi_ctx* src = nullptr, hipStream_t build_stream = nullptr, bool lazy = false);
+void finish_level(fi_ctx* level);
+void join_levels(fi_ctx* c);
+void abandon_levels(fi_ctx* c);
+void close_assemble_timing(fi_ctx* root);
+void close_levels(fi_ctx* root, fi_ctx* top, int code, const std::string& msg);
 fi_ctx* twin_prepare(fi_ctx* c);
 void twin_assemble(fi_ctx* c, hipStream_t build_stream);
 void twin_assemble_lumped(fi_ctx* c);
@@ -674,7 +680,13 @@
 	CgScalars end()
 	{
 		FI_HIP_TRY(hipEventRecord(timer.e1, st));
-		FI_HIP_TRY(hipEventSynchronize(timer.e1));
+		if (c0->store_dst) {
+			store_solution_async(c0);
+			c0->store_enqueued = true;
+			FI_HIP_TRY(hipStreamSynchronize(st));
+		} else {
+			FI_HIP_TRY(hipEventSynchronize(timer.e1));
+		}
 		FI_HIP_TRY(hipEventElapsedTime(&ms, timer.e0, timer.e1));
 		return *c0->scal_host;
 	}
@@ -704,6 +716,7 @@
 			residual_rule_stats(c->stats);
 			if (h.done == 4) {
 				FI_HIP_TRY(hipMemsetAsync(c->x.p, 0, sizeof(T) * c->g.nloc, c->stream));
+				c->store_enqueued = false;
 			}
 		}
 	}
diff --git a/include/fi_hip.h b/include/fi_hip.h
--- a/include/fi_hip.h
+++ b/include/fi_hip.h
@@ -183,6 +183,7 @@
 int fi_get_Atb_f64(fi_ctx* ctx, double* out);
 int fi_get_diag_f64(fi_ctx* ctx, double* out);
 int fi_get_stats(const fi_ctx* ctx, fi_stats* out);
+int fi_levels_pending(const fi_ctx* ctx, int* count);
 int fi_memory_pool(long long keep_bytes, long long* cached_bytes);
 int fi_time_apply(fi_ctx* ctx, int reps, double* ms_per_launch);
 
```

Result: no change. 1.876 billion (median of 6 runs) (+0.9%).
